# valeoai/rainbow-iqn-apex

Hardware: NVIDIA H100
Metric: learner grad-steps/sec (batch=512, N=N'=64) (higher is better)
Workload: dtype fp16 fwd / bf16 bwd tensor-core products, fp32 accumulate; fp32 elsewhere

## Files before the change

### include/riqn_b200.h

```cpp
#ifndef RIQN_B200_H
#define RIQN_B200_H

#ifdef __cplusplus
extern "C" {
#endif

#define RIQN_B200_ABI_VERSION 1

int riqn_version(void);
long long riqn_launch_count(void);
int riqn_device_ok(void);

typedef struct riqn_dyn_state {
  unsigned long long rng_offset;
  float adam_neg_step_size;
  float adam_sqrt_bc2;
  double is_capacity;
  double is_beta;
} riqn_dyn_state;

typedef struct riqn_conv_geom {
  int B, Cin, H, W;
  int Cout, KH, KW;
  int stride, pad;
  int OH, OW;
  long in_bstride;
} riqn_conv_geom;


int riqn_conv_fwd(const riqn_conv_geom* g, const void* in, int in_is_u8, const float* w, const float* bias,
                  float* col, float* out, void* stream);
int riqn_conv_bwd(const riqn_conv_geom* g, const float* dout, const float* out, const float* col, const float* w,
                  float* dY, float* dcol, float* dw, float* dbias, float* din, void* stream);

int riqn_im2col_f32(const riqn_conv_geom* g, const void* in, int in_is_u8, float* col, void* stream);

int riqn_conv_fwd_tc(const riqn_conv_geom* g, const void* in, int in_is_u8, const void* w_hi, const void* w_lo,
                     const float* bias, void* col_hi, void* col_lo, void* colT_hi, float* out, void* stream);
int riqn_s2d_u8(const riqn_conv_geom* g, const unsigned char* in, void* a_px, void* stream);
int riqn_random_shift(int B, int C, int H, int W, const void* in0, long in0_bstride, const void* in1, long in1_bstride,
                      int is_u8, const int* shifts, void* out, void* stream);
int riqn_conv_fwd_strip(const riqn_conv_geom* g, const void* a_hi, const void* a_lo, const void* w_hi, const void* w_lo,
                        const float* bias, float* out, void* next_hi, void* next_lo, int next_stride, int next_grid,
                        const void* w2_hi, const void* w2_lo, const float* bias2, int share_a, void* stream);
int riqn_conv_bwd_strip(const riqn_conv_geom* g, const float* dout, const float* out, const void* a_hi, const void* w_hi,
                        const int* perm, void* dYg, float* dwp_scratch, float* dw, float* dbias, float* din,
                        float wgrad_scale, void* stream);

int riqn_conv_bwd_tc(const riqn_conv_geom* g, const float* dout, const float* out, const void* colT_hi, const void* wT_hi,
                     void* dY_hi, void* dYT_hi, float* dcol, float* dw, float* dbias, float* din, float wgrad_scale,
                     void* stream);
int riqn_split_bf16_scaled(long rows, int cols, const float* src, float scale, void* hi, void* lo, void* stream);

int riqn_fill_uniform(long n, unsigned long long seed, unsigned long long stream_id, float* out,
                      const riqn_dyn_state* dyn, void* stream);

#define RIQN_RISK_NEUTRAL 0
#define RIQN_RISK_CVAR 1
#define RIQN_RISK_WANG 2
#define RIQN_RISK_CPW 3
#define RIQN_RISK_POW 4
#define RIQN_RISK_NORM 5
int riqn_fill_tau_distorted(long n, unsigned long long seed, unsigned long long stream_id, int measure, float eta,
                            float* out, const riqn_dyn_state* dyn, void* stream);
int riqn_noisy_sample(long n, unsigned long long seed, unsigned long long stream_id, float* out,
                      const riqn_dyn_state* dyn, void* stream);
int riqn_fill_shifts(long n, int pad, unsigned long long seed, unsigned long long stream_id, int* out,
                     const riqn_dyn_state* dyn, void* stream);

int riqn_noisy_compose(int out_features, int in_features, const float* weight_mu, const float* weight_sigma,
                       float* weight_epsilon, const float* eps_in, const float* eps_out, const float* bias_mu,
                       const float* bias_sigma, float* bias_epsilon, float* w_eff, float* b_eff, int training,
                       void* stream);

typedef struct riqn_noisy_layer {
  int out_features, in_features;
  const float* weight_mu;
  const float* weight_sigma;
  float* weight_epsilon;
  const float* bias_mu;
  const float* bias_sigma;
  float* bias_epsilon;
  float* eps_in;
  float* eps_out;
  float* w_eff;
  float* b_eff;
  unsigned long long stream_in, stream_out;
  void* w_hi;
  void* w_lo;
  int w_fp16;
} riqn_noisy_layer;

int riqn_noisy_reset_net(int n_layers, const riqn_noisy_layer* layers, unsigned long long seed, int sample, int training,
                         const riqn_dyn_state* dyn, void* stream);
int riqn_noisy_linear_fwd(long rows, int in_features, int out_features, const float* x, const float* w_eff,
                          const float* b_eff, float* h, void* stream);
int riqn_noisy_linear_dgrad(long rows, int in_features, int out_features, const float* dh, const float* w_eff,
                            float* dx, void* stream);
int riqn_noisy_linear_wgrad(long rows, int in_features, int out_features, const float* dh, const float* x,
                            const float* weight_epsilon, const float* bias_epsilon, float* db_scratch,
                            float* grad_weight_mu, float* grad_weight_sigma, float* grad_bias_mu,
                            float* grad_bias_sigma, void* stream);

int riqn_noisy_bias_grad(long rows, int out_features, const float* dh, const float* bias_epsilon, float* db_scratch,
                         float* grad_bias_mu, float* grad_bias_sigma, void* stream);

int riqn_quantile_embed_fwd(int batch, int num_quantiles, int embed_dim, int feat_dim, const float* tau,
                            const float* feat, const float* iqn_w, const float* iqn_b, float* cosv, float* x,
                            void* stream);
int riqn_quantile_embed_bwd(int batch, int num_quantiles, int embed_dim, int feat_dim, const float* x,
                            const float* feat, const float* cosv, float* dx_inout, float* dfeat, float* grad_iqn_w,
                            float* grad_iqn_b, void* stream);

int riqn_quantile_embed_fwd_tc(int batch, int num_quantiles, int embed_dim, int feat_dim, const float* tau,
                               const float* feat, const void* iqn_w_hi, const void* iqn_w_lo, const float* iqn_b,
                               void* cos_hi, void* cos_lo, void* cos_t_hi, float* x32, void* x_hi, void* x_lo, void* x_hi_t,
                               void* x_lo_t, int x_fp16, void* stream);
int riqn_quantile_embed_bwd_tc(int batch, int num_quantiles, int embed_dim, int feat_dim, const void* x_hi, const void* x_lo,
                               const float* feat, const void* cos_hi, const void* dx, int dx_is_bf16, void* dpre,
                               float* dfeat, float* grad_iqn_w, float* grad_iqn_b, void* stream);

int riqn_dueling_fwd(long rows, int batch, int hidden, int action_space, const float* h, const float* wz,
                     const float* bz, float* q, void* stream);
int riqn_dueling_bwd(long rows, int batch, int hidden, int action_space, const float* h, const float* wz,
                     const float* dtheta, const float* gscale, float gscale_mul, const long long* actions, float* dh,
                     float* dz, void* dz_bf16, void* stream);
int riqn_dueling_bwd_bf16(long rows, int batch, int hidden, int action_space, const float* h, const void* h_bf16,
                          const float* wz,
                          const float* dtheta, const float* gscale, float gscale_mul, const long long* actions, void* dh_hi,
                          void* dh_hi_t,
                          float* dh_colsum, float* dz, void* dz_bf16, void* stream);
int riqn_dueling_bwd_dense(long rows, int batch, int hidden, int action_space, const float* h, const float* wz,
                           const float* grad_q, float* dh, float* dz, void* dz_bf16, void* stream);
int riqn_dueling_bwd_dense_bf16(long rows, int batch, int hidden, int action_space, const float* h, const void* h_bf16,
                                const float* wz, const float* grad_q, void* dh_hi, void* dh_hi_t, float* dh_colsum,
                                float* dz, void* dz_bf16, void* stream);
int riqn_z_wgrad_tc(long rows, int hidden, int action_space, const void* dz_bf16, const void* h_bf16, const float* dz,
                    float* dwz_scratch, float* dbz_scratch, const float* eps_w_zv, const float* eps_b_zv,
                    const float* eps_w_za, const float* eps_b_za, float* g_mu_zv, float* g_sig_zv, float* g_bmu_zv,
                    float* g_bsig_zv, float* g_mu_za, float* g_sig_za, float* g_bmu_za, float* g_bsig_za, void* stream);
int riqn_z_wgrad(long rows, int hidden, int action_space, const float* dz, const float* h, float* dwz_scratch,
                 float* dbz_scratch, const float* eps_w_zv, const float* eps_b_zv, const float* eps_w_za,
                 const float* eps_b_za, float* g_mu_zv, float* g_sig_zv, float* g_bmu_zv, float* g_bsig_zv,
                 float* g_mu_za, float* g_sig_za, float* g_bmu_za, float* g_bsig_za, void* stream);

int riqn_argmax_mean(int batch, int num_quantiles, int action_space, const float* q, long long* a_star, void* stream);
int riqn_iqn_loss_fwd_bwd(int batch, int n_tau, int n_tau_prime, int action_space, const float* q_online,
                          const float* q_target, const float* tau, const long long* actions, const long long* a_star,
                          const float* returns, const float* nonterminals, float gamma_n, float kappa, float* loss,
                          float* dtheta, float* theta_out, float* target_out, void* stream);
int riqn_miqn_loss_fwd_bwd(int batch, int n_tau, int n_tau_prime, int action_space, const float* q_online,
                           const float* q_target, const float* tau, const long long* actions, const float* returns,
                           const float* nonterminals, float gamma_n, float kappa, float alpha, float entropy_tau, float l0,
                           float* loss, float* dtheta, float* theta_out, float* target_out, float* bonus_out, void* stream);

int riqn_value_rescale(long n, const float* x, float eps, int inverse, float* out, void* stream);
int riqn_iqn_loss_fwd_bwd_h(int batch, int n_tau, int n_tau_prime, int action_space, const float* q_online,
                            const float* q_target, const float* tau, const long long* actions, const long long* a_star,
                            const float* returns, const float* nonterminals, float gamma_n, float kappa, float eps,
                            float* loss, float* dtheta, float* theta_out, float* target_out, void* stream);
int riqn_argmax_expected_h(int batch, int n, int action_space, const float* q, const float* w, float eps, float* values,
                           long long* a_star, void* stream);

int riqn_fqf_fractions(int batch, int n, const float* logits, float* tau, float* tau_hat, float* dtau, float* entropy,
                       void* stream);
int riqn_fqf_fraction_bwd(int batch, int n, int action_space, const float* logits, const float* tau, const float* q_hat,
                          const float* q_bnd, const long long* actions, const float* gscale, float gscale_mul,
                          float entropy_coef, float* dlogits, float* loss_out, void* stream);
int riqn_fqf_fraction_wgrad(int batch, int n, int feat_dim, const float* dlogits, const float* feat, float* grad_w,
                            float* grad_b, void* stream);
int riqn_argmax_weighted(int batch, int n, int action_space, const float* q, const float* w, long long* a_star,
                         void* stream);

int riqn_c51_head_fwd(int batch, int action_space, int atoms, const float* zv, const float* za, const float* support,
                      float* p, float* logp, long long* a_star, void* stream);
int riqn_c51_loss_fwd_bwd(int batch, int action_space, int atoms, const float* logp_online, const float* p_target,
                          const long long* actions, const long long* a_star, const float* returns,
                          const float* nonterminals, const float* support, float gamma_n, float v_min, float v_max,
                          float delta_z, float* loss, float* dq, float* m_out, void* stream);
int riqn_c51_loss_fwd_bwd_h(int batch, int action_space, int atoms, const float* logp_online, const float* p_target,
                            const long long* actions, const long long* a_star, const float* returns,
                            const float* nonterminals, const float* support, float gamma_n, float v_min, float v_max,
                            float delta_z, float eps, float* loss, float* dq, float* m_out, void* stream);
int riqn_c51_head_bwd(int batch, int action_space, int atoms, const float* dq, const float* gscale, float gscale_mul,
                      const long long* actions, float* dzv, float* dza, void* stream);
int riqn_c51_head_bwd_dense(int batch, int action_space, int atoms, const float* out, const float* grad_out, int is_log,
                            float* dzv, float* dza, void* stream);

int riqn_qr_head_fwd(int batch, int action_space, int n, const float* zv, const float* za, float* q, void* stream);
int riqn_qr_head_bwd(int batch, int action_space, int n, const float* dtheta, const float* gscale, float gscale_mul,
                     const long long* actions, float* dzv, float* dza, void* stream);
int riqn_qr_head_bwd_dense(int batch, int action_space, int n, const float* grad_q, float* dzv, float* dza, void* stream);
int riqn_zero_f32(float* p, long n, void* stream);
int riqn_relu_mask(long n, const float* act, float* grad, void* stream);
int riqn_linear_fwd_ld(long rows, int in_features, int out_features, const float* x, long ldx, const float* w,
                       const float* bias, float* y, long ldy, int relu, void* stream);
int riqn_linear_dgrad_ld(long rows, int in_features, int out_features, const float* dy, long lddy, const float* w,
                         float* dx, long lddx, void* stream);
int riqn_noisy_wgrad_ld(long rows, int in_features, int out_features, const float* dy, long lddy, const float* x, long ldx,
                        const float* weight_epsilon, float* grad_mu, float* grad_sigma, void* stream);

int riqn_adam_step(long n, float* params, const float* grads, float* exp_avg, float* exp_avg_sq, int step, float lr,
                   float beta1, float beta2, float eps, float grad_scale, const riqn_dyn_state* dyn, void* stream);

int riqn_sumtree_stratified(int n, unsigned long long seed, unsigned long long stream_id, const double* tree,
                            double* values, const riqn_dyn_state* dyn, void* stream);
int riqn_sumtree_sample(int n, long capacity, int actor_capacity, const double* tree, const double* values,
                        const long long* index_actor, int history, int n_step, long long* tree_idx,
                        long long* data_idx, double* priorities, void* stream);
int riqn_sumtree_is_weights(int n, const double* tree, const double* priorities, double current_capacity,
                            double priority_weight, double* w64, float* w32, int* n_nonpositive,
                            const riqn_dyn_state* dyn, void* stream);
int riqn_sumtree_update(int n, long capacity, double* tree, const long long* tree_idx, const float* loss,
                        float priority_exponent, int apply_pow, float* new_priorities, double* diff_scratch,
                        double* max_priority, void* stream);

int riqn_replay_append(int n, int actor_capacity, int id_actor, int start, const unsigned char* frames,
                       const int* timestep, const int* action, const float* reward, const unsigned char* nonterminal,
                       unsigned char* s_frames, int* s_timestep, int* s_action, float* s_reward,
                       unsigned char* s_nonterminal, void* stream);
int riqn_frame_gather(int batch, int actor_capacity, int history, int n_step, const long long* data_idx,
                      const unsigned char* s_frames, const int* s_timestep, const int* s_action, const float* s_reward,
                      const unsigned char* s_nonterminal, const double* gamma_pow, unsigned char* window,
                      long long* actions, float* returns, float* nonterminals, void* stream);

int riqn_split_bf16(long rows, int cols, const float* src, void* hi, void* lo, void* hi_t, void* lo_t, int fp16, void* stream);
typedef struct riqn_split_job {
  const float* src;
  const int* perm;
  int rows, cols;
  float div;
  void* hi;
  void* lo;
  void* hi_t;
} riqn_split_job;
int riqn_split_bf16_multi(int n_jobs, const riqn_split_job* jobs, void* stream);
int riqn_gemm_bf16_tc(int M, int N, int K, const void* a_hi, const void* a_lo, const void* b_hi, const void* b_lo,
                      float* c, long ldc, int epilogue, const float* bias, float* out2, const float* eps, int split_k,
                      void* c_t_bf16, void* c_bf16, int fmt, void* stream);
int riqn_gemm_bf16_tc_mn(int M, int N, int K, const void* a, const void* b_kn, int a_is_km, float* c, long ldc, int epilogue,
                         float* out2, const float* eps, float alpha, int split_k, void* c_bf16, int fmt, void* stream);

int riqn_gemm_f32(int M, int N, int K, const float* A, long sAm, long sAk, const float* B, long sBn, long sBk,
                  float* C, long ldc, void* stream);

#ifdef __cplusplus
}
#endif
#endif
```

### rainbow_iqn_apex_b200/_lib.py

```python
import ctypes as C
import os

import torch

HERE = os.path.dirname(os.path.abspath(__file__))
LIB_PATH = os.path.join(HERE, "libriqn_b200.so")

c_f32p = C.c_void_p
_P = C.c_void_p


class ConvGeom(C.Structure):
    _fields_ = [("B", C.c_int), ("Cin", C.c_int), ("H", C.c_int), ("W", C.c_int), ("Cout", C.c_int),
                ("KH", C.c_int), ("KW", C.c_int), ("stride", C.c_int), ("pad", C.c_int), ("OH", C.c_int),
                ("OW", C.c_int), ("in_bstride", C.c_long)]


class NoisyLayer(C.Structure):
    _fields_ = [("out_features", C.c_int), ("in_features", C.c_int), ("weight_mu", _P), ("weight_sigma", _P),
                ("weight_epsilon", _P), ("bias_mu", _P), ("bias_sigma", _P), ("bias_epsilon", _P), ("eps_in", _P),
                ("eps_out", _P), ("w_eff", _P), ("b_eff", _P), ("stream_in", C.c_ulonglong),
                ("stream_out", C.c_ulonglong), ("w_hi", _P), ("w_lo", _P), ("w_fp16", C.c_int)]


class SplitJob(C.Structure):
    _fields_ = [("src", _P), ("perm", _P), ("rows", C.c_int), ("cols", C.c_int), ("div", C.c_float), ("hi", _P),
                ("lo", _P), ("hi_t", _P)]


SIGNATURES = {
    "riqn_version": [],
    "riqn_device_ok": [],
    "riqn_launch_count": [],
    "riqn_conv_fwd": [C.POINTER(ConvGeom), _P, C.c_int, _P, _P, _P, _P, _P],
    "riqn_conv_bwd": [C.POINTER(ConvGeom), _P, _P, _P, _P, _P, _P, _P, _P, _P, _P],
    "riqn_im2col_f32": [C.POINTER(ConvGeom), _P, C.c_int, _P, _P],
    "riqn_conv_fwd_tc": [C.POINTER(ConvGeom), _P, C.c_int, _P, _P, _P, _P, _P, _P, _P, _P],
    "riqn_conv_bwd_tc": [C.POINTER(ConvGeom), _P, _P, _P, _P, _P, _P, _P, _P, _P, _P, C.c_float, _P],
    "riqn_s2d_u8": [C.POINTER(ConvGeom), _P, _P, _P],
    "riqn_conv_fwd_strip": [C.POINTER(ConvGeom), _P, _P, _P, _P, _P, _P, _P, _P, C.c_int, C.c_int, _P, _P, _P, C.c_int, _P],
    "riqn_conv_bwd_strip": [C.POINTER(ConvGeom), _P, _P, _P, _P, _P, _P, _P, _P, _P, _P, C.c_float, _P],
    "riqn_split_bf16_scaled": [C.c_long, C.c_int, _P, C.c_float, _P, _P, _P],
    "riqn_fill_uniform": [C.c_long, C.c_ulonglong, C.c_ulonglong, _P, _P, _P],
    "riqn_fill_tau_distorted": [C.c_long, C.c_ulonglong, C.c_ulonglong, C.c_int, C.c_float, _P, _P, _P],
    "riqn_noisy_sample": [C.c_long, C.c_ulonglong, C.c_ulonglong, _P, _P, _P],
    "riqn_fill_shifts": [C.c_long, C.c_int, C.c_ulonglong, C.c_ulonglong, _P, _P, _P],
    "riqn_random_shift": [C.c_int] * 4 + [_P, C.c_long, _P, C.c_long, C.c_int, _P, _P, _P],
    "riqn_noisy_compose": [C.c_int, C.c_int, _P, _P, _P, _P, _P, _P, _P, _P, _P, _P, C.c_int, _P],
    "riqn_noisy_reset_net": [C.c_int, C.POINTER(NoisyLayer), C.c_ulonglong, C.c_int, C.c_int, _P, _P],
    "riqn_noisy_linear_fwd": [C.c_long, C.c_int, C.c_int, _P, _P, _P, _P, _P],
    "riqn_noisy_linear_dgrad": [C.c_long, C.c_int, C.c_int, _P, _P, _P, _P],
    "riqn_noisy_linear_wgrad": [C.c_long, C.c_int, C.c_int, _P, _P, _P, _P, _P, _P, _P, _P, _P, _P],
    "riqn_noisy_bias_grad": [C.c_long, C.c_int, _P, _P, _P, _P, _P, _P],
    "riqn_quantile_embed_fwd": [C.c_int, C.c_int, C.c_int, C.c_int, _P, _P, _P, _P, _P, _P, _P],
    "riqn_quantile_embed_fwd_tc": [C.c_int, C.c_int, C.c_int, C.c_int] + [_P] * 13 + [C.c_int, _P],
    "riqn_quantile_embed_bwd_tc": [C.c_int, C.c_int, C.c_int, C.c_int, _P, _P, _P, _P, _P, C.c_int, _P, _P, _P, _P, _P],
    "riqn_quantile_embed_bwd": [C.c_int, C.c_int, C.c_int, C.c_int, _P, _P, _P, _P, _P, _P, _P, _P],
    "riqn_dueling_fwd": [C.c_long, C.c_int, C.c_int, C.c_int, _P, _P, _P, _P, _P],
    "riqn_dueling_bwd": [C.c_long, C.c_int, C.c_int, C.c_int, _P, _P, _P, _P, C.c_float, _P, _P, _P, _P, _P],
    "riqn_dueling_bwd_bf16": [C.c_long, C.c_int, C.c_int, C.c_int] + [_P] * 5 + [C.c_float] + [_P] * 7,
    "riqn_dueling_bwd_dense": [C.c_long, C.c_int, C.c_int, C.c_int, _P, _P, _P, _P, _P, _P, _P],
    "riqn_dueling_bwd_dense_bf16": [C.c_long, C.c_int, C.c_int, C.c_int] + [_P] * 10,
    "riqn_z_wgrad": [C.c_long, C.c_int, C.c_int] + [_P] * 17,
    "riqn_z_wgrad_tc": [C.c_long, C.c_int, C.c_int] + [_P] * 18,
    "riqn_argmax_mean": [C.c_int, C.c_int, C.c_int, _P, _P, _P],
    "riqn_iqn_loss_fwd_bwd": [C.c_int, C.c_int, C.c_int, C.c_int, _P, _P, _P, _P, _P, _P, _P, C.c_float, C.c_float,
                              _P, _P, _P, _P, _P],
    "riqn_miqn_loss_fwd_bwd": [C.c_int] * 4 + [_P] * 6 + [C.c_float] * 5 + [_P] * 6,
    "riqn_fqf_fractions": [C.c_int, C.c_int] + [_P] * 6,
    "riqn_fqf_fraction_bwd": [C.c_int] * 3 + [_P] * 6 + [C.c_float] * 2 + [_P] * 3,
    "riqn_fqf_fraction_wgrad": [C.c_int] * 3 + [_P] * 5,
    "riqn_argmax_weighted": [C.c_int] * 3 + [_P] * 4,
    "riqn_c51_head_fwd":[C.c_int, C.c_int, C.c_int, _P, _P, _P, _P, _P, _P, _P],
    "riqn_c51_loss_fwd_bwd": [C.c_int, C.c_int, C.c_int, _P, _P, _P, _P, _P, _P, _P, C.c_float, C.c_float, C.c_float,
                              C.c_float, _P, _P, _P, _P],
    "riqn_value_rescale": [C.c_long, _P, C.c_float, C.c_int, _P, _P],
    "riqn_iqn_loss_fwd_bwd_h": [C.c_int] * 4 + [_P] * 7 + [C.c_float] * 3 + [_P] * 5,
    "riqn_argmax_expected_h": [C.c_int] * 3 + [_P, _P, C.c_float, _P, _P, _P],
    "riqn_c51_loss_fwd_bwd_h": [C.c_int] * 3 + [_P] * 7 + [C.c_float] * 5 + [_P] * 4,
    "riqn_c51_head_bwd": [C.c_int, C.c_int, C.c_int, _P, _P, C.c_float, _P, _P, _P, _P],
    "riqn_c51_head_bwd_dense": [C.c_int, C.c_int, C.c_int, _P, _P, C.c_int, _P, _P, _P],
    "riqn_qr_head_fwd": [C.c_int] * 3 + [_P] * 4,
    "riqn_qr_head_bwd": [C.c_int] * 3 + [_P, _P, C.c_float, _P, _P, _P, _P],
    "riqn_qr_head_bwd_dense": [C.c_int] * 3 + [_P] * 4,
    "riqn_zero_f32": [_P, C.c_long, _P],
    "riqn_relu_mask": [C.c_long, _P, _P, _P],
    "riqn_linear_fwd_ld": [C.c_long, C.c_int, C.c_int, _P, C.c_long, _P, _P, _P, C.c_long, C.c_int, _P],
    "riqn_linear_dgrad_ld": [C.c_long, C.c_int, C.c_int, _P, C.c_long, _P, _P, C.c_long, _P],
    "riqn_noisy_wgrad_ld": [C.c_long, C.c_int, C.c_int, _P, C.c_long, _P, C.c_long, _P, _P, _P, _P],
    "riqn_adam_step": [C.c_long, _P, _P, _P, _P, C.c_int, C.c_float, C.c_float, C.c_float, C.c_float, C.c_float, _P, _P],
    "riqn_sumtree_stratified": [C.c_int, C.c_ulonglong, C.c_ulonglong, _P, _P, _P, _P],
    "riqn_sumtree_sample": [C.c_int, C.c_long, C.c_int, _P, _P, _P, C.c_int, C.c_int, _P, _P, _P, _P],
    "riqn_sumtree_is_weights": [C.c_int, _P, _P, C.c_double, C.c_double, _P, _P, _P, _P, _P],
    "riqn_sumtree_update": [C.c_int, C.c_long, _P, _P, _P, C.c_float, C.c_int, _P, _P, _P, _P],
    "riqn_replay_append": [C.c_int, C.c_int, C.c_int, C.c_int] + [_P] * 11,
    "riqn_frame_gather": [C.c_int, C.c_int, C.c_int, C.c_int] + [_P] * 12,
    "riqn_split_bf16_multi": [C.c_int, C.POINTER(SplitJob), _P],
    "riqn_split_bf16": [C.c_long, C.c_int, _P, _P, _P, _P, _P, C.c_int, _P],
    "riqn_gemm_bf16_tc": [C.c_int, C.c_int, C.c_int, _P, _P, _P, _P, _P, C.c_long, C.c_int, _P, _P, _P, C.c_int, _P, _P, C.c_int, _P],
    "riqn_gemm_bf16_tc_mn": [C.c_int, C.c_int, C.c_int, _P, _P, C.c_int, _P, C.c_long, C.c_int, _P, _P, C.c_float, C.c_int, _P, C.c_int, _P],
    "riqn_gemm_f32": [C.c_int, C.c_int, C.c_int, _P, C.c_long, C.c_long, _P, C.c_long, C.c_long, _P, C.c_long, _P],
}

_lib = None


class RiqnError(RuntimeError):
    pass


def load():
    global _lib
    if _lib is not None:
        return _lib
    if not os.path.exists(LIB_PATH):
        raise RiqnError(f"{LIB_PATH} is missing: build it with `python -c 'import __graft_entry__ as g; g.build()'` "
                        "(the product has no CPU or PyTorch fallback)")
    lib = C.CDLL(LIB_PATH)
    for name, argtypes in SIGNATURES.items():
        fn = getattr(lib, name)
        fn.argtypes = argtypes
        fn.restype = C.c_longlong if name == "riqn_launch_count" else C.c_int
    if lib.riqn_version() != 1:
        raise RiqnError("ABI version mismatch between _lib.py and libriqn_b200.so")
    _lib = lib
    return lib


def stream():
    return torch.cuda.current_stream().cuda_stream


def ptr(t):
    if t is None:
        return None
    return t.data_ptr()


_timers = None


def time_entry_points(names):
    global _timers
    _timers = {n: [] for n in names} if names else None
    return _timers


def call(name, *args):
    lib = load()
    if _timers is not None and name in _timers:
        e0, e1 = torch.cuda.Event(enable_timing=True), torch.cuda.Event(enable_timing=True)
        e0.record()
        rc = getattr(lib, name)(*args, stream())
        e1.record()
        _timers[name].append((e0, e1, args))
    else:
        rc = getattr(lib, name)(*args, stream())
    if rc != 0:
        raise RiqnError(f"{name} failed with cudaError {rc}")


def launch_count():
    return int(load().riqn_launch_count())


def require_device():
    if not torch.cuda.is_available():
        raise RiqnError("rainbow_iqn_apex_b200 needs a CUDA device (H100, sm_90a); there is no CPU path")
    lib = load()
    ok = lib.riqn_device_ok()
    if ok != 1:
        raise RiqnError(f"libriqn_b200.so holds sm_90a code only; riqn_device_ok() returned {ok}")
```

### rainbow_iqn_apex_b200/c51.py

```python
import torch

from ._lib import call, ptr
from .model import FEAT


def _tc_mode(B):
    from .model import PRECISION
    return PRECISION["fwd"] != "fp32" and PRECISION["bwd"] == "bf16" and B % 8 == 0


def forward(net, x, log=False, keep=None, fresh_weights=False, want_argmax=None, support=None):
    if not fresh_weights:
        net._compose_weights()
    zv, za = hidden_z(net, x, keep=keep)
    B, A, atoms = zv.shape[0], net.action_space, net.atoms
    out = torch.empty(B, A, atoms, device=zv.device)
    if support is None:
        support = net._support(zv.device)
    call("riqn_c51_head_fwd", B, A, atoms, ptr(zv), ptr(za), ptr(support), None if log else ptr(out),
         ptr(out) if log else None, ptr(want_argmax))
    return out


def hidden_z(net, x, keep=None, col_cache=None, feat=None):
    from .model import PRECISION
    if feat is None:
        feat = net.trunk(x, keep, col_cache)
    B = feat.shape[0]
    dev = feat.device
    hid = net.hidden
    nzv, nza = net.fcnoisy_z_v.out_features, net.fcnoisy_z_a.out_features
    h = torch.empty(B, 2 * hid, device=dev)
    x_bf = None
    if _tc_mode(B):
        fwd = PRECISION["fwd"]
        f16, x3 = fwd == "fp16", fwd == "bf16x3"
        x_hi = torch.empty(B, FEAT, dtype=torch.float16 if f16 else torch.bfloat16, device=dev)
        x_lo = torch.empty(B, FEAT, dtype=torch.bfloat16, device=dev) if (x3 or (f16 and keep is not None)) else None
        call("riqn_split_bf16", B, FEAT, ptr(feat), ptr(x_hi), ptr(x_lo), None, None, 1 if f16 else 0)
        call("riqn_gemm_bf16_tc", B, 2 * hid, FEAT, ptr(x_hi), ptr(x_lo) if x3 else None, ptr(net._w_hi),
             ptr(net._w_lo) if x3 else None, ptr(h), 2 * hid, 1, ptr(net._b_eff_h), None, None, 1, None, None, 3 if f16 else 0)
        x_bf = x_lo if f16 else x_hi
    else:
        call("riqn_noisy_linear_fwd", B, FEAT, 2 * hid, ptr(feat), ptr(net._w_eff_h), ptr(net._b_eff_h), ptr(h))
    zv = torch.empty(B, nzv, device=dev)
    za = torch.empty(B, nza, device=dev)
    wz, bz = net._w_eff_z, net._b_eff_z
    hv, ha = h[:, :hid], h[:, hid:]
    call("riqn_linear_fwd_ld", B, hid, nzv, ptr(hv), 2 * hid, ptr(wz), ptr(bz), ptr(zv), nzv, 0)
    wza, bza = wz[nzv:], bz[nzv:]
    call("riqn_linear_fwd_ld", B, hid, nza, ptr(ha), 2 * hid, ptr(wza), ptr(bza), ptr(za), nza, 0)
    if keep is not None:
        keep.update(feat=feat, h=h, B=B, x_bf=x_bf)
    return zv, za


def loss_core(agent, states, actions, returns, next_states, nonterminals, debug=None):
    from .compute_loss_iqn import _as_device_inputs
    states, actions, returns, next_states, nonterminals = _as_device_inputs(
        agent, states, actions, returns, next_states, nonterminals)
    on, tg = agent.online_net, agent.target_net
    B, A, atoms = states.shape[0], agent.action_space, agent.atoms
    dev = states.device
    inj = getattr(agent, "_inject", None)
    if isinstance(inj, list):
        inj = inj.pop(0) if inj else None
    noises = inj.get("noises", (None, None, None)) if inj else (None, None, None)
    on.reset_noise(noises[1])
    a_star = torch.empty(B, dtype=torch.int64, device=dev)
    forward(on, next_states, fresh_weights=True, want_argmax=a_star, support=agent.acting_support)
    tg.reset_noise(noises[2])
    pns = forward(tg, next_states, fresh_weights=True, support=agent.support)
    on.reset_noise(noises[0])
    keep = {}
    log_ps = forward(on, states, log=True, keep=keep, fresh_weights=True, support=agent.support)
    loss = torch.empty(B, device=dev)
    dq = torch.empty(B, atoms, device=dev)
    m_out = torch.empty(B, atoms, device=dev) if debug is not None else None
    args = (ptr(log_ps), ptr(pns), ptr(actions), ptr(a_star), ptr(returns), ptr(nonterminals), ptr(agent.support),
            float(agent.discount ** agent.n), float(agent.Vmin), float(agent.Vmax), float(agent.delta_z))
    eps = getattr(agent, "value_rescaling", None)
    if eps is None:
        call("riqn_c51_loss_fwd_bwd", B, A, atoms, *args, ptr(loss), ptr(dq), ptr(m_out))
    else:
        call("riqn_c51_loss_fwd_bwd_h", B, A, atoms, *args, eps, ptr(loss), ptr(dq), ptr(m_out))
    if debug is not None:
        debug.update(a_star=a_star, m=m_out, log_ps=log_ps)
    version = getattr(on, "_noise_version", 0)

    def backward(gscale, gscale_mul=1.0):
        if getattr(on, "_noise_version", 0) != version:
            raise RuntimeError("the online network's noise was resampled between the C51 loss and its backward")
        gscale = gscale.contiguous().float()
        dzv = torch.empty(B, atoms, device=dev)
        dza = torch.empty(B, A * atoms, device=dev)
        call("riqn_c51_head_bwd", B, A, atoms, ptr(dq), ptr(gscale), float(gscale_mul), ptr(actions), ptr(dzv), ptr(dza))
        _backward_below_head(on, keep, dzv, dza, on.grad_view)

    return loss, backward


def backward_dense(on, keep, out, grad_out, log, gv):
    B, A, atoms = out.shape
    dzv = torch.empty(B, atoms, device=out.device)
    dza = torch.empty(B, A * atoms, device=out.device)
    call("riqn_c51_head_bwd_dense", B, A, atoms, ptr(out), ptr(grad_out), 1 if log else 0, ptr(dzv), ptr(dza))
    _backward_below_head(on, keep, dzv, dza, gv)


def _backward_below_head(on, keep, dzv, dza, gv):
    B, dev = keep["B"], dzv.device
    hid = on.hidden
    hvL, haL, zvL, zaL = on.fcnoisy_h_v, on.fcnoisy_h_a, on.fcnoisy_z_v, on.fcnoisy_z_a
    h = keep["h"]
    dh = torch.empty(B, 2 * hid, device=dev)
    dhv, dha = dh[:, :hid], dh[:, hid:]
    hv, ha = h[:, :hid], h[:, hid:]
    nzv, nza = zvL.out_features, zaL.out_features
    w_z = on._w_eff_z
    wzv, wza = w_z[:nzv], w_z[nzv:]
    call("riqn_linear_dgrad_ld", B, hid, nzv, ptr(dzv), nzv, ptr(wzv), ptr(dhv), 2 * hid)
    call("riqn_linear_dgrad_ld", B, hid, nza, ptr(dza), nza, ptr(wza), ptr(dha), 2 * hid)
    call("riqn_relu_mask", dh.numel(), ptr(h), ptr(dh))
    scratch = torch.empty(max(nza, 2 * hid), device=dev)
    for layer, d, xin in ((zvL, dzv, hv), (zaL, dza, ha)):
        call("riqn_noisy_wgrad_ld", B, hid, layer.out_features, ptr(d), layer.out_features, ptr(xin), 2 * hid,
             ptr(layer.weight_epsilon), ptr(gv(layer.weight_mu)), ptr(gv(layer.weight_sigma)))
        call("riqn_noisy_bias_grad", B, layer.out_features, ptr(d), ptr(layer.bias_epsilon), ptr(scratch),
             ptr(gv(layer.bias_mu)), ptr(gv(layer.bias_sigma)))
    dfeat = torch.empty(B, FEAT, device=dev)
    if keep.get("x_bf") is not None:
        from .model import PRECISION
        dh_bf = torch.empty(B, 2 * hid, dtype=torch.bfloat16, device=dev)
        call("riqn_split_bf16", B, 2 * hid, ptr(dh), ptr(dh_bf), None, None, None, 0)
        w_bf = on._w_lo if PRECISION["fwd"] == "fp16" else on._w_hi
        call("riqn_gemm_bf16_tc_mn", 2 * hid, FEAT, B, ptr(dh_bf), ptr(keep["x_bf"]), 1, ptr(gv(hvL.weight_mu)), FEAT, 3,
             ptr(gv(hvL.weight_sigma)), ptr(hvL.weight_epsilon), 1.0, 1, None, 0)
        call("riqn_noisy_bias_grad", B, 2 * hid, ptr(dh), ptr(hvL.bias_epsilon), ptr(scratch), ptr(gv(hvL.bias_mu)),
             ptr(gv(hvL.bias_sigma)))
        call("riqn_gemm_bf16_tc_mn", B, FEAT, 2 * hid, ptr(dh_bf), ptr(w_bf), 0, ptr(dfeat), FEAT, 0, None, None, 1.0, 1,
             None, 0)
    else:
        call("riqn_noisy_linear_wgrad", B, FEAT, 2 * hid, ptr(dh), ptr(keep["feat"]), ptr(hvL.weight_epsilon),
             ptr(hvL.bias_epsilon), ptr(scratch), ptr(gv(hvL.weight_mu)), ptr(gv(hvL.weight_sigma)), ptr(gv(hvL.bias_mu)),
             ptr(gv(hvL.bias_sigma)))
        call("riqn_noisy_linear_dgrad", B, FEAT, 2 * hid, ptr(dh), ptr(on._w_eff_h), ptr(dfeat))
    on.backward_trunk(keep, dfeat)


class _HeadLoss(torch.autograd.Function):

    @staticmethod
    def forward(ctx, core, agent, states, actions, returns, next_states, nonterminals, debug, *params):
        loss, bw = core(agent, states, actions, returns, next_states, nonterminals, debug=debug)
        ctx.bw, ctx.n_params = bw, len(params)
        return loss

    @staticmethod
    def backward(ctx, grad_loss):
        ctx.bw(grad_loss)
        ctx.bw = None
        return (None,) * (8 + ctx.n_params)


def compute_loss_c51(agent, states, actions, returns, next_states, nonterminals, debug=None):
    if torch.is_grad_enabled():
        params = [p for p in agent.online_net.parameters() if p.requires_grad]
        return _HeadLoss.apply(loss_core, agent, states, actions, returns, next_states, nonterminals, debug, *params)
    loss, _ = loss_core(agent, states, actions, returns, next_states, nonterminals, debug=debug)
    return loss
```

### rainbow_iqn_apex_b200/compute_loss_iqn.py

```python
import ctypes
import math
import numbers

import torch

from ._lib import call, ptr

MUNCHAUSEN_DEFAULTS = {"munchausen_alpha": 0.9, "munchausen_tau": 0.03, "munchausen_l0": -1.0}


def check_munchausen(munchausen, alpha=0.9, entropy_tau=0.03, l0=-1.0, rainbow_only=False, risk=None):
    if isinstance(munchausen, bool) or (isinstance(munchausen, numbers.Integral) and munchausen in (0, 1)):
        if not munchausen:
            return None
    else:
        raise ValueError(f"munchausen must be 0 or 1, got {munchausen!r}")
    vals = []
    for name, v, ok, need in (("munchausen_alpha", alpha, lambda x: x >= 0.0, ">= 0"),
                              ("munchausen_tau", entropy_tau, lambda x: x > 0.0, "> 0"),
                              ("munchausen_l0", l0, lambda x: x <= 0.0, "<= 0")):
        if isinstance(v, bool) or not isinstance(v, numbers.Real):
            raise ValueError(f"{name} must be a real number, got {v!r}")
        f = ctypes.c_float(v).value
        if not (math.isfinite(f) and ok(f)):
            raise ValueError(f"{name} must be finite and {need} (as a float32), got {v!r}")
        vals.append(float(v))
    if rainbow_only:
        raise ValueError("Munchausen targets are implemented for the IQN loss; rainbow_only (C51) does not take them")
    if risk is not None:
        raise ValueError("Munchausen targets have no target action a* to act risk-sensitively on: use the neutral measure")
    return tuple(vals)


VALUE_RESCALING_DEFAULTS = {"value_rescaling_eps": 1e-3}


def check_value_rescaling(value_rescaling, eps=1e-3, munchausen=None):
    if isinstance(value_rescaling, bool) or (isinstance(value_rescaling, numbers.Integral) and value_rescaling in (0, 1)):
        if not value_rescaling:
            return None
    else:
        raise ValueError(f"value_rescaling must be 0 or 1, got {value_rescaling!r}")
    if isinstance(eps, bool) or not isinstance(eps, numbers.Real):
        raise ValueError(f"value_rescaling_eps must be a real number, got {eps!r}")
    f = ctypes.c_float(eps).value
    if not (math.isfinite(f) and f >= 0.0):
        raise ValueError(f"value_rescaling_eps must be finite and >= 0 (as a float32), got {eps!r}")
    if munchausen is not None:
        raise ValueError("value rescaling and Munchausen targets do not combine: set value_rescaling = 0 or munchausen = 0")
    return float(eps)


def greedy_actions(agent, batch, n, q, w=None):
    A = agent.action_space
    a_star = torch.empty(batch, dtype=torch.int64, device=q.device)
    eps = getattr(agent, "value_rescaling", None)
    if eps is not None:
        call("riqn_argmax_expected_h", batch, n, A, ptr(q), ptr(w), eps, None, ptr(a_star))
    elif w is None:
        call("riqn_argmax_mean", batch, n, A, ptr(q), ptr(a_star))
    else:
        call("riqn_argmax_weighted", batch, n, A, ptr(q), ptr(w), ptr(a_star))
    return a_star


def _quantile_loss(agent, B, N, Np, q_on, q_tgt, tau, actions, a_star, returns, nonterminals, loss, dtheta, theta_out,
                   target_out):
    args = (ptr(q_on), ptr(q_tgt), ptr(tau), ptr(actions), ptr(a_star), ptr(returns), ptr(nonterminals),
            float(agent.discount ** agent.n), float(agent.kappa))
    outs = (ptr(loss), ptr(dtheta), ptr(theta_out), ptr(target_out))
    eps = getattr(agent, "value_rescaling", None)
    if eps is None:
        call("riqn_iqn_loss_fwd_bwd", B, N, Np, agent.action_space, *args, *outs)
    else:
        call("riqn_iqn_loss_fwd_bwd_h", B, N, Np, agent.action_space, *args, eps, *outs)


def _as_device_inputs(agent, states, actions, returns, next_states, nonterminals):
    dev = agent.online_net._flat.device

    def frames(x):
        x = x.to(dev)
        return x if x.dtype == torch.uint8 else x.float()

    return (frames(states), actions.to(dev, torch.int64).contiguous(), returns.to(dev, torch.float32).contiguous(),
            frames(next_states), nonterminals.to(dev, torch.float32).contiguous())


def loss_core(agent, states, actions, returns, next_states, nonterminals, keep_graph=True, debug=None):
    states, actions, returns, next_states, nonterminals = _as_device_inputs(
        agent, states, actions, returns, next_states, nonterminals)
    on, tg = agent.online_net, agent.target_net
    B = states.shape[0]
    K, Np, N = agent.num_quantile_samples, agent.num_tau_prime_samples, agent.num_tau_samples
    inj = getattr(agent, "_inject", None)
    if isinstance(inj, list):
        inj = inj.pop(0) if inj else None
    noises = inj.get("noises", (None, None, None)) if inj else (None, None, None)
    taus = inj.get("taus", (None, None, None)) if inj else (None, None, None)
    dev = states.device
    if getattr(agent, "munchausen", None) is not None:
        return _munchausen_core(agent, states, actions, returns, next_states, nonterminals, noises, taus, keep_graph, debug)
    if getattr(agent, "fqf", None) is not None:
        return _fqf_core(agent, states, actions, returns, next_states, nonterminals, noises, keep_graph, debug)

    on.reset_noise(noises[0])
    cache = {}
    pair = on.trunk_pair(tg, next_states) if not on.rainbow_only else None
    f_on, f_tg = pair if pair is not None else (None, None)
    q_sel, tau_sel = on.forward(next_states, K, tau=taus[0], fresh_weights=True, col_cache=cache, feat=f_on,
                                risk=getattr(agent, "risk", None))
    a_star = greedy_actions(agent, B, K, q_sel)
    tg.reset_noise(noises[1])
    q_tgt, _ = tg.forward(next_states, Np, tau=taus[1], fresh_weights=True, col_cache=cache, feat=f_tg)
    on.reset_noise(noises[2])
    keep = {} if keep_graph else None
    q_on, tau = on.forward(states, N, tau=taus[2], keep=keep, fresh_weights=True)

    loss = torch.empty(B, device=dev)
    dtheta = torch.empty(N * B, device=dev)
    theta_out = target_out = None
    if debug is not None:
        theta_out = torch.empty(B, N, device=dev)
        target_out = torch.empty(B, Np, device=dev)
    _quantile_loss(agent, B, N, Np, q_on, q_tgt, tau, actions, a_star, returns, nonterminals, loss, dtheta, theta_out,
                   target_out)
    if debug is not None:
        debug.update(a_star=a_star, theta=theta_out, target=target_out, q_sel=q_sel, q_tgt=q_tgt, q_on=q_on, tau=tau,
                     keep=keep, tau_sel=tau_sel)
    return loss, dtheta, keep, actions


def _munchausen_core(agent, states, actions, returns, next_states, nonterminals, noises, taus, keep_graph, debug):
    on, tg = agent.online_net, agent.target_net
    B, A = states.shape[0], agent.action_space
    Np, N = agent.num_tau_prime_samples, agent.num_tau_samples
    alpha, entropy_tau, l0 = agent.munchausen
    dev = states.device
    tg.reset_noise(noises[0])
    q_tgt, _ = tg.forward(torch.cat((next_states, states)), Np, tau=taus[0], fresh_weights=True)
    on.reset_noise(noises[1])
    keep = {} if keep_graph else None
    q_on, tau = on.forward(states, N, tau=taus[1], keep=keep, fresh_weights=True)

    loss = torch.empty(B, device=dev)
    dtheta = torch.empty(N * B, device=dev)
    theta_out = target_out = bonus_out = None
    if debug is not None:
        theta_out = torch.empty(B, N, device=dev)
        target_out = torch.empty(B, Np, device=dev)
        bonus_out = torch.empty(B, device=dev)
    call("riqn_miqn_loss_fwd_bwd", B, N, Np, A, ptr(q_on), ptr(q_tgt), ptr(tau), ptr(actions), ptr(returns),
         ptr(nonterminals), float(agent.discount ** agent.n), float(agent.kappa), alpha, entropy_tau, l0, ptr(loss),
         ptr(dtheta), ptr(theta_out), ptr(target_out), ptr(bonus_out))
    if debug is not None:
        debug.update(bonus=bonus_out, theta=theta_out, target=target_out, q_tgt=q_tgt, q_on=q_on, tau=tau, keep=keep)
    return loss, dtheta, keep, actions


def _fqf_core(agent, states, actions, returns, next_states, nonterminals, noises, keep_graph, debug):
    on, tg, fnet = agent.online_net, agent.target_net, agent.fraction_net
    B, N = states.shape[0], agent.num_tau_samples
    dev = states.device
    on.reset_noise(noises[0])
    cache = {}
    pair = on.trunk_pair(tg, next_states)
    f_on, f_tg = pair if pair is not None else (on.trunk(next_states, col_cache=cache), None)
    fr_n = fnet.propose(f_on)
    q_sel, _ = on.forward(next_states, N, tau=fr_n["tau_hat"], fresh_weights=True, col_cache=cache, feat=f_on)
    a_star = greedy_actions(agent, B, N, q_sel, fr_n["dtau"])
    keep = {} if keep_graph else None
    feat = on.trunk(states, keep)
    fr = fnet.propose(feat)
    tg.reset_noise(noises[1])
    q_tgt, _ = tg.forward(next_states, N, tau=fr["tau_hat"], fresh_weights=True, col_cache=cache, feat=f_tg)
    on.reset_noise(noises[2])
    q_on, tau_hat = on.forward(states, N, tau=fr["tau_hat"], keep=keep, fresh_weights=True, feat=feat)
    nb = N - 1 if (N - 1) * B % 2 == 0 else N
    q_bnd, _ = on.forward(states, nb, tau=fr["tau"][:, 1:nb + 1].t().contiguous(), fresh_weights=True, feat=feat)

    loss = torch.empty(B, device=dev)
    dtheta = torch.empty(N * B, device=dev)
    theta_out = target_out = None
    if debug is not None:
        theta_out = torch.empty(B, N, device=dev)
        target_out = torch.empty(B, N, device=dev)
    _quantile_loss(agent, B, N, N, q_on, q_tgt, tau_hat, actions, a_star, returns, nonterminals, loss, dtheta, theta_out,
                   target_out)
    if keep is not None:
        keep["fqf"] = dict(fr=fr, q_hat=q_on, q_bnd=q_bnd, actions=actions, debug=debug)
    if debug is not None:
        debug.update(a_star=a_star, theta=theta_out, target=target_out, q_sel=q_sel, q_tgt=q_tgt, q_on=q_on, q_bnd=q_bnd,
                     tau=fr["tau"], tau_hat=fr["tau_hat"], dtau=fr["dtau"], logits=fr["logits"], entropy=fr["entropy"],
                     tau_next=fr_n["tau"], dtau_next=fr_n["dtau"], keep=keep)
    return loss, dtheta, keep, actions


def fraction_backward(agent, keep, gscale, gscale_mul=1.0):
    fk = keep.get("fqf") if keep is not None else None
    if fk is None:
        return
    dlogits, floss = agent.fraction_net.backward(fk["fr"], fk["q_hat"], fk["q_bnd"], fk["actions"], gscale, gscale_mul,
                                                 agent.fqf[1])
    if fk["debug"] is not None:
        fk["debug"].update(dlogits=dlogits, fraction_loss=floss)


class _IQNLoss(torch.autograd.Function):
    @staticmethod
    def forward(ctx, agent, states, actions, returns, next_states, nonterminals, debug, *params):
        loss, dtheta, keep, actions = loss_core(agent, states, actions, returns, next_states, nonterminals,
                                                keep_graph=True, debug=debug)
        ctx.agent, ctx.keep, ctx.dtheta, ctx.actions = agent, keep, dtheta, actions
        ctx.n_params = len(params)
        return loss

    @staticmethod
    def backward(ctx, grad_loss):
        g = grad_loss.contiguous().float()
        ctx.agent.online_net.backward_iqn(ctx.keep, ctx.dtheta, g, ctx.actions)
        fraction_backward(ctx.agent, ctx.keep, g)
        ctx.keep = None
        return (None,) * (7 + ctx.n_params)


def compute_loss_actor_or_learner_iqn(agent, states, actions, returns, next_states, nonterminals, debug=None):
    if torch.is_grad_enabled():
        params = [p for p in agent.online_net.parameters() if p.requires_grad]
        return _IQNLoss.apply(agent, states, actions, returns, next_states, nonterminals, debug, *params)
    loss, _, _, _ = loss_core(agent, states, actions, returns, next_states, nonterminals, keep_graph=False, debug=debug)
    return loss
```

### rainbow_iqn_apex_b200/csrc/conv.cu

```cuda
#include "common.cuh"
#include "gemm.h"
#include "../../include/riqn_b200.h"

namespace riqn {

template <typename T>
__device__ __forceinline__ float load_px(const T* p);
template <>
__device__ __forceinline__ float load_px<uint8_t>(const uint8_t* p) { return (float)(*p) / 255.0f; }
template <>
__device__ __forceinline__ float load_px<float>(const float* p) { return *p; }

template <typename T>
__global__ void im2col_kernel(riqn_conv_geom g, const T* __restrict__ in, float* __restrict__ col) {
  const int K = g.Cin * g.KH * g.KW;
  const long total = (long)g.B * g.OH * g.OW * K;
  for (long idx = (long)blockIdx.x * blockDim.x + threadIdx.x; idx < total; idx += (long)gridDim.x * blockDim.x) {
    const int k = (int)(idx % K);
    const long m = idx / K;
    const int kw = k % g.KW, kh = (k / g.KW) % g.KH, c = k / (g.KW * g.KH);
    const int ow = (int)(m % g.OW), oh = (int)((m / g.OW) % g.OH), b = (int)(m / ((long)g.OW * g.OH));
    const int ih = oh * g.stride + kh - g.pad, iw = ow * g.stride + kw - g.pad;
    float v = 0.f;
    if (ih >= 0 && ih < g.H && iw >= 0 && iw < g.W) v = load_px<T>(&in[(long)b * g.in_bstride + ((long)c * g.H + ih) * g.W + iw]);
    col[idx] = v;
  }
}

__global__ void conv_dy_kernel(int B, int Cout, int ohw, const float* __restrict__ dout,
                               const float* __restrict__ out, float* __restrict__ dY) {
  const long total = (long)B * Cout * ohw;
  for (long idx = (long)blockIdx.x * blockDim.x + threadIdx.x; idx < total; idx += (long)gridDim.x * blockDim.x) {
    const int p = (int)(idx % ohw);
    const int c = (int)((idx / ohw) % Cout);
    const long b = idx / ((long)ohw * Cout);
    const float v = out[idx] > 0.f ? dout[idx] : 0.f;
    dY[(b * ohw + p) * Cout + c] = v;
  }
}

__global__ void col2im_kernel(riqn_conv_geom g, const float* __restrict__ dcol, float* __restrict__ din) {
  const int K = g.Cin * g.KH * g.KW;
  const long total = (long)g.B * g.Cin * g.H * g.W;
  for (long idx = (long)blockIdx.x * blockDim.x + threadIdx.x; idx < total; idx += (long)gridDim.x * blockDim.x) {
    const int iw = (int)(idx % g.W), ih = (int)((idx / g.W) % g.H);
    const int c = (int)((idx / ((long)g.W * g.H)) % g.Cin);
    const long b = idx / ((long)g.W * g.H * g.Cin);
    float acc = 0.f;
    for (int kh = 0; kh < g.KH; ++kh) {
      const int t = ih + g.pad - kh;
      if (t < 0 || t % g.stride) continue;
      const int oh = t / g.stride;
      if (oh >= g.OH) continue;
      for (int kw = 0; kw < g.KW; ++kw) {
        const int u = iw + g.pad - kw;
        if (u < 0 || u % g.stride) continue;
        const int ow = u / g.stride;
        if (ow >= g.OW) continue;
        acc += dcol[((b * g.OH + oh) * g.OW + ow) * K + (c * g.KH + kh) * g.KW + kw];
      }
    }
    din[idx] = acc;
  }
}

__global__ void col2im_tile_kernel(riqn_conv_geom g, int CC, const float* __restrict__ dcol, float* __restrict__ din) {
  extern __shared__ float acc[];
  const int K = g.Cin * g.KH * g.KW, khw = g.KH * g.KW, ohw = g.OH * g.OW, hw = g.H * g.W;
  const int chunks = g.Cin / CC;
  const long b = blockIdx.x / chunks;
  const int c0 = (blockIdx.x % chunks) * CC;
  for (int i = threadIdx.x; i < CC * hw; i += blockDim.x) acc[i] = 0.f;
  __syncthreads();
  const int per_row = CC * khw;
  const float* base = dcol + b * ohw * (long)K + (long)c0 * khw;
  for (int e = threadIdx.x; e < ohw * per_row; e += blockDim.x) {
    const int m = e / per_row, j = e - m * per_row;
    const int c = j / khw, r = j - c * khw;
    const int kh = r / g.KW, kw = r - kh * g.KW;
    const int oh = m / g.OW, ow = m - oh * g.OW;
    const int ih = oh * g.stride + kh - g.pad, iw = ow * g.stride + kw - g.pad;
    if (ih >= 0 && ih < g.H && iw >= 0 && iw < g.W) atomicAdd(&acc[c * hw + ih * g.W + iw], base[(long)m * K + j]);
  }
  __syncthreads();
  float* out = din + (b * g.Cin + c0) * hw;
  for (int i = threadIdx.x; i < CC * hw; i += blockDim.x) out[i] = acc[i];
}

static int col2im(const riqn_conv_geom* g, const float* dcol, float* din, cudaStream_t s) {
  const int hw = g->H * g->W;
  int CC = g->Cin;
  while (CC > 1 && ((long)CC * hw * 4 > 16 * 1024 || g->Cin % CC)) --CC;
  if ((long)CC * hw * 4 <= 48 * 1024) {
    col2im_tile_kernel<<<g->B * (g->Cin / CC), 256, (size_t)CC * hw * 4, s>>>(*g, CC, dcol, din);
  } else {
    long total = (long)g->B * g->Cin * hw;
    long blocks = (total + 255) / 256;
    col2im_kernel<<<(int)(blocks > 32L * riqn_sms() ? 32L * riqn_sms() : blocks), 256, 0, s>>>(*g, dcol, din);
  }
  return (int)cudaGetLastError();
}

__global__ void colsum_part_kernel(long M, int N, const float* __restrict__ X, float* __restrict__ part, int rows_per_block) {
  __shared__ float upper[128];
  const int n = blockIdx.x * 128 + (threadIdx.x & 127);
  const int half = threadIdx.x >> 7;
  const long r0 = (long)blockIdx.y * rows_per_block;
  const long r1 = min(M, r0 + rows_per_block);
  float acc = 0.f;
  if (n < N)
    for (long r = r0 + half; r < r1; r += 2) acc += X[r * N + n];
  if (half) upper[threadIdx.x & 127] = acc;
  __syncthreads();
  if (!half && n < N) part[(long)blockIdx.y * N + n] = acc + upper[threadIdx.x];
}

int colsum_add(long M, int N, const float* X, float* out, cudaStream_t s) {
  int rows_per_block = 256;
  dim3 grid((N + 127) / 128, (unsigned)((M + rows_per_block - 1) / rows_per_block));
  StreamScratch part;
  RIQN_CUDA(part.alloc((size_t)grid.y * N, s));
  colsum_part_kernel<<<grid, 256, 0, s>>>(M, N, X, part.p, rows_per_block);
  RIQN_LAUNCH_CHECK();
  return sum_slots_add((int)grid.y, N, part.p, out, s);
}

using bf16 = __nv_bfloat16;

template <typename T>
__device__ __forceinline__ float im2col_at(const riqn_conv_geom& g, const T* __restrict__ in, long m, int k) {
  const int kw = k % g.KW, kh = (k / g.KW) % g.KH, c = k / (g.KW * g.KH);
  const int ow = (int)(m % g.OW), oh = (int)((m / g.OW) % g.OH);
  const long b = m / ((long)g.OW * g.OH);
  const int ih = oh * g.stride + kh - g.pad, iw = ow * g.stride + kw - g.pad;
  if (ih < 0 || ih >= g.H || iw < 0 || iw >= g.W) return 0.f;
  return load_px<T>(&in[b * g.in_bstride + ((long)c * g.H + ih) * g.W + iw]);
}

__device__ __forceinline__ void pack8(const float (&x)[8], uint4& hi, uint4& lo) {
  uint32_t h[4], l[4];
#pragma unroll
  for (int t = 0; t < 8; t += 2) {
    const bf16 h0 = __float2bfloat16_rn(x[t]), h1 = __float2bfloat16_rn(x[t + 1]);
    const bf16 l0 = __float2bfloat16_rn(x[t] - __bfloat162float(h0)), l1 = __float2bfloat16_rn(x[t + 1] - __bfloat162float(h1));
    h[t / 2] = (uint32_t)__bfloat16_as_ushort(h0) | ((uint32_t)__bfloat16_as_ushort(h1) << 16);
    l[t / 2] = (uint32_t)__bfloat16_as_ushort(l0) | ((uint32_t)__bfloat16_as_ushort(l1) << 16);
  }
  hi = make_uint4(h[0], h[1], h[2], h[3]);
  lo = make_uint4(l[0], l[1], l[2], l[3]);
}

template <typename T>
__global__ void im2col_bf16_kernel(riqn_conv_geom g, const T* __restrict__ in, bf16* __restrict__ hi, bf16* __restrict__ lo) {
  const int K = g.Cin * g.KH * g.KW, K8 = K / 8;
  const long total = (long)g.B * g.OH * g.OW * K8;
  for (long idx = (long)blockIdx.x * blockDim.x + threadIdx.x; idx < total; idx += (long)gridDim.x * blockDim.x) {
    const int k0 = (int)(idx % K8) * 8;
    const long m = idx / K8;
    const int ow = (int)(m % g.OW), oh = (int)((m / g.OW) % g.OH);
    const long b = m / ((long)g.OW * g.OH);
    int kw = k0 % g.KW, kh = (k0 / g.KW) % g.KH, c = k0 / (g.KW * g.KH);
    const T* base = in + b * g.in_bstride;
    const int ih0 = oh * g.stride - g.pad, iw0 = ow * g.stride - g.pad;
    float x[8];
#pragma unroll
    for (int t = 0; t < 8; ++t) {
      const int ih = ih0 + kh, iw = iw0 + kw;
      x[t] = (ih >= 0 && ih < g.H && iw >= 0 && iw < g.W) ? load_px<T>(&base[((long)c * g.H + ih) * g.W + iw]) : 0.f;
      if (++kw == g.KW) { kw = 0; if (++kh == g.KH) { kh = 0; ++c; } }
    }
    uint4 h, l;
    pack8(x, h, l);
    *reinterpret_cast<uint4*>(hi + m * K + k0) = h;
    if (lo) *reinterpret_cast<uint4*>(lo + m * K + k0) = l;
  }
}

__global__ void im2col_bf16_u8_kernel(riqn_conv_geom g, const uint8_t* __restrict__ in, bf16* __restrict__ hi, bf16* __restrict__ lo) {
  __shared__ uint32_t lut[256];
  {
    const float x = (float)threadIdx.x / 255.0f;
    const bf16 h = __float2bfloat16_rn(x);
    const bf16 l = __float2bfloat16_rn(x - __bfloat162float(h));
    if (threadIdx.x < 256) lut[threadIdx.x] = (uint32_t)__bfloat16_as_ushort(h) | ((uint32_t)__bfloat16_as_ushort(l) << 16);
  }
  __syncthreads();
  const int K = g.Cin * g.KH * g.KW, K8 = K / 8;
  const long total = (long)g.B * g.OH * g.OW * K8;
  for (long idx = (long)blockIdx.x * blockDim.x + threadIdx.x; idx < total; idx += (long)gridDim.x * blockDim.x) {
    const int k0 = (int)(idx % K8) * 8;
    const long m = idx / K8;
    const int ow = (int)(m % g.OW), oh = (int)((m / g.OW) % g.OH);
    const long b = m / ((long)g.OW * g.OH);
    int kw = k0 % g.KW, kh = (k0 / g.KW) % g.KH, c = k0 / (g.KW * g.KH);
    const uint8_t* base = in + b * g.in_bstride;
    const int ih0 = oh * g.stride - g.pad, iw0 = ow * g.stride - g.pad;
    uint32_t e[8];
#pragma unroll
    for (int t = 0; t < 8; ++t) {
      const int ih = ih0 + kh, iw = iw0 + kw;
      e[t] = (ih >= 0 && ih < g.H && iw >= 0 && iw < g.W) ? lut[base[((long)c * g.H + ih) * g.W + iw]] : 0u;
      if (++kw == g.KW) { kw = 0; if (++kh == g.KH) { kh = 0; ++c; } }
    }
    uint4 h, l;
    h.x = (e[0] & 0xffffu) | (e[1] << 16); h.y = (e[2] & 0xffffu) | (e[3] << 16);
    h.z = (e[4] & 0xffffu) | (e[5] << 16); h.w = (e[6] & 0xffffu) | (e[7] << 16);
    l.x = (e[0] >> 16) | (e[1] & 0xffff0000u); l.y = (e[2] >> 16) | (e[3] & 0xffff0000u);
    l.z = (e[4] >> 16) | (e[5] & 0xffff0000u); l.w = (e[6] >> 16) | (e[7] & 0xffff0000u);
    *reinterpret_cast<uint4*>(hi + m * K + k0) = h;
    if (lo) *reinterpret_cast<uint4*>(lo + m * K + k0) = l;
  }
}

__global__ void __launch_bounds__(256) im2col_f32_staged_kernel(riqn_conv_geom g, const float* __restrict__ in,
                                                                bf16* __restrict__ hi, bf16* __restrict__ lo) {
  extern __shared__ __align__(16) uint32_t simg[];
  const int chw = g.Cin * g.H * g.W, K = g.Cin * g.KH * g.KW, K8 = K / 8, ohw = g.OH * g.OW;
  const long b = blockIdx.x;
  const float4* src = reinterpret_cast<const float4*>(in + b * g.in_bstride);
  for (int i = threadIdx.x; i < chw / 4; i += blockDim.x) {
    const float4 v = __ldg(src + i);
    const float x[4] = {v.x, v.y, v.z, v.w};
    uint32_t w[4];
#pragma unroll
    for (int t = 0; t < 4; ++t) {
      const bf16 h = __float2bfloat16_rn(x[t]);
      const bf16 l = __float2bfloat16_rn(x[t] - __bfloat162float(h));
      w[t] = (uint32_t)__bfloat16_as_ushort(h) | ((uint32_t)__bfloat16_as_ushort(l) << 16);
    }
    reinterpret_cast<uint4*>(simg)[i] = make_uint4(w[0], w[1], w[2], w[3]);
  }
  __syncthreads();
  const int hw = g.H * g.W;
  for (int item = threadIdx.x; item < ohw * K8; item += blockDim.x) {
    const int m = item / K8, k0 = (item - m * K8) * 8;
    const int oh = m / g.OW, ow = m - oh * g.OW;
    int kw = k0 % g.KW, kh = (k0 / g.KW) % g.KH, c = k0 / (g.KW * g.KH);
    const int ih0 = oh * g.stride - g.pad, iw0 = ow * g.stride - g.pad;
    uint32_t e[8];
#pragma unroll
    for (int t = 0; t < 8; ++t) {
      const int ih = ih0 + kh, iw = iw0 + kw;
      e[t] = ((unsigned)ih < (unsigned)g.H && (unsigned)iw < (unsigned)g.W) ? simg[c * hw + ih * g.W + iw] : 0u;
      if (++kw == g.KW) { kw = 0; if (++kh == g.KH) { kh = 0; ++c; } }
    }
    const long o = (b * ohw + m) * K + k0;
    *reinterpret_cast<uint4*>(hi + o) = make_uint4(__byte_perm(e[0], e[1], 0x5410), __byte_perm(e[2], e[3], 0x5410),
                                                   __byte_perm(e[4], e[5], 0x5410), __byte_perm(e[6], e[7], 0x5410));
    if (lo)
      *reinterpret_cast<uint4*>(lo + o) = make_uint4(__byte_perm(e[0], e[1], 0x7632), __byte_perm(e[2], e[3], 0x7632),
                                                     __byte_perm(e[4], e[5], 0x7632), __byte_perm(e[6], e[7], 0x7632));
  }
}

template <typename T>
__global__ void im2col_bf16_t_kernel(riqn_conv_geom g, const T* __restrict__ in, bf16* __restrict__ hiT) {
  const int K = g.Cin * g.KH * g.KW;
  const long M = (long)g.B * g.OH * g.OW, M8 = M / 8;
  const long total = M8 * K;
  for (long idx = (long)blockIdx.x * blockDim.x + threadIdx.x; idx < total; idx += (long)gridDim.x * blockDim.x) {
    const long m0 = (idx % M8) * 8;
    const int k = (int)(idx / M8);
    const int kw = k % g.KW, kh = (k / g.KW) % g.KH, c = k / (g.KW * g.KH);
    int ow = (int)(m0 % g.OW), oh = (int)((m0 / g.OW) % g.OH);
    long b = m0 / ((long)g.OW * g.OH);
    float x[8];
#pragma unroll
    for (int t = 0; t < 8; ++t) {
      const int ih = oh * g.stride + kh - g.pad, iw = ow * g.stride + kw - g.pad;
      x[t] = (ih >= 0 && ih < g.H && iw >= 0 && iw < g.W)
                 ? load_px<T>(&in[b * g.in_bstride + ((long)c * g.H + ih) * g.W + iw]) : 0.f;
      if (++ow == g.OW) { ow = 0; if (++oh == g.OH) { oh = 0; ++b; } }
    }
    uint4 h, l;
    pack8(x, h, l);
    *reinterpret_cast<uint4*>(hiT + (long)k * M + m0) = h;
  }
}

__global__ void conv_dy_bf16_kernel(int B, int Cout, int ohw, const float* __restrict__ dout, const float* __restrict__ out,
                                    bf16* __restrict__ dY, bf16* __restrict__ dYT, float* __restrict__ dbias_part) {
  const int c = blockIdx.y;
  const long M = (long)B * ohw;
  float acc = 0.f;
  for (long i = (long)blockIdx.x * blockDim.x + threadIdx.x; i < M; i += (long)gridDim.x * blockDim.x) {
    const long b = i / ohw;
    const int p = (int)(i - b * ohw);
    const long src = (b * Cout + c) * ohw + p;
    const float v = out[src] > 0.f ? dout[src] : 0.f;
    acc += v;
    const bf16 h = __float2bfloat16_rn(v);
    if (dY) dY[i * Cout + c] = h;
    dYT[(long)c * M + i] = h;
  }
  acc = warp_sum(acc);
  __shared__ float red[32];
  if ((threadIdx.x & 31) == 0) red[threadIdx.x >> 5] = acc;
  __syncthreads();
  if (threadIdx.x < 32) {
    float v = threadIdx.x < (blockDim.x >> 5) ? red[threadIdx.x] : 0.f;
    v = warp_sum(v);
    if (threadIdx.x == 0) dbias_part[(long)blockIdx.x * Cout + c] = v;
  }
}

__global__ void __launch_bounds__(256) conv_dy_tile_kernel(int B, int Cout, int ohw, const float* __restrict__ dout,
                                                           const float* __restrict__ out, bf16* __restrict__ dY,
                                                           bf16* __restrict__ dYT, float* __restrict__ dbias_part) {
  __shared__ __align__(16) unsigned short tile[64][66];
  __shared__ float bsum[64];
  const long M = (long)B * ohw;
  const int lane = threadIdx.x & 31, warp = threadIdx.x >> 5;
  if (threadIdx.x < 64) bsum[threadIdx.x] = 0.f;
  __syncthreads();
  const long n_tiles = (M + 63) / 64;
  for (long tix = blockIdx.x; tix < n_tiles; tix += gridDim.x) {
    const long m0 = tix * 64;
    long src0[2];
    bool ok[2];
#pragma unroll
    for (int h = 0; h < 2; ++h) {
      const long m = m0 + lane + 32 * h;
      ok[h] = m < M;
      const long b = ok[h] ? m / ohw : 0;
      src0[h] = b * Cout * ohw + (ok[h] ? m - b * ohw : 0);
    }
    for (int c = warp; c < Cout; c += 8) {
      float acc = 0.f;
#pragma unroll
      for (int h = 0; h < 2; ++h) {
        float v = 0.f;
        if (ok[h]) {
          const long src = src0[h] + (long)c * ohw;
          v = out[src] > 0.f ? dout[src] : 0.f;
        }
        const bf16 hb = __float2bfloat16_rn(v);
        if (ok[h]) dYT[(long)c * M + m0 + lane + 32 * h] = hb;
        tile[lane + 32 * h][c] = __bfloat16_as_ushort(hb);
        acc += v;
      }
      acc = warp_sum(acc);
      if (lane == 0) bsum[c] += acc;
    }
    __syncthreads();
    if (dY) {
      const int ppr = Cout >> 3;
      for (int idx = threadIdx.x; idx < 64 * ppr; idx += blockDim.x) {
        const int r = idx / ppr, pc = idx - r * ppr;
        if (m0 + r < M) {
          const uint32_t* w = reinterpret_cast<const uint32_t*>(&tile[r][pc * 8]);
          *reinterpret_cast<uint4*>(dY + (m0 + r) * Cout + pc * 8) = make_uint4(w[0], w[1], w[2], w[3]);
        }
      }
    }
    __syncthreads();
  }
  if (threadIdx.x < Cout) dbias_part[(long)blockIdx.x * Cout + threadIdx.x] = bsum[threadIdx.x];
}

__global__ void __launch_bounds__(256) s2d_u8_kernel(riqn_conv_geom g, int G, const uint8_t* __restrict__ in,
                                                     bf16* __restrict__ a_px) {
  extern __shared__ __align__(16) uint8_t img[];
  const int chw = g.Cin * g.H * g.W, s = g.stride, ss = s * s, Kc = ss * g.Cin, K8 = Kc / 8;
  const long b = blockIdx.x;
  const uint4* src = reinterpret_cast<const uint4*>(in + b * g.in_bstride);
  for (int i = threadIdx.x; i < chw / 16; i += blockDim.x) reinterpret_cast<uint4*>(img)[i] = src[i];
  __syncthreads();
  const bool fast = s == 4 && g.pad == 1 && (g.W & 3) == 0 && (G - 1) * 4 + 2 < g.W && (G - 1) * 4 + 2 < g.H;
  if (fast) {
    const uint32_t* img32 = reinterpret_cast<const uint32_t*>(img);
    const int wpr = g.W >> 2;
    auto cvt2 = [](uint32_t w, uint32_t sa, uint32_t sb) -> uint32_t {
      const float fa = __uint_as_float(__byte_perm(w, 0x4B000000u, sa)) - 8388608.0f;
      const float fb = __uint_as_float(__byte_perm(w, 0x4B000000u, sb)) - 8388608.0f;
      return __byte_perm(__float_as_uint(fa), __float_as_uint(fb), 0x7632);
    };
    for (int item = threadIdx.x; item < G * G * K8; item += blockDim.x) {
      const int r = item / K8, q = item - r * K8;
      const int gy = r / G, gx = r - gy * G, c = q >> 1, iy0 = (q & 1) * 2;
      uint32_t o[4];
#pragma unroll
      for (int h = 0; h < 2; ++h) {
        const int y = gy * 4 + iy0 + h - 1;
        uint32_t w0 = 0u, w1 = 0u;
        if (y >= 0) {
          const uint32_t* rowp = img32 + (c * g.H + y) * wpr + gx;
          w0 = gx > 0 ? rowp[-1] : 0u;
          w1 = rowp[0];
        }
        const uint32_t a = __byte_perm(w0, w1, 0x0043);
        o[2 * h] = cvt2(a, 0x7650, 0x7651);
        o[2 * h + 1] = cvt2(w1, 0x7651, 0x7652);
      }
      *reinterpret_cast<uint4*>(a_px + (b * G * G + r) * Kc + q * 8) = make_uint4(o[0], o[1], o[2], o[3]);
    }
    return;
  }
  for (int item = threadIdx.x; item < G * G * K8; item += blockDim.x) {
    const int r = item / K8, k0 = (item - r * K8) * 8;
    const int gy = r / G, gx = r - gy * G;
    uint32_t e[8];
#pragma unroll
    for (int t = 0; t < 8; ++t) {
      const int k = k0 + t, c = k / ss, rem = k - c * ss, iy = rem / s, ix = rem - iy * s;
      const int y = gy * s + iy - g.pad, x = gx * s + ix - g.pad;
      e[t] = ((unsigned)y < (unsigned)g.H && (unsigned)x < (unsigned)g.W)
                 ? __float_as_uint((float)img[(c * g.H + y) * g.W + x]) >> 16 : 0u;
    }
    *reinterpret_cast<uint4*>(a_px + (b * G * G + r) * Kc + k0) =
        make_uint4(e[0] | (e[1] << 16), e[2] | (e[3] << 16), e[4] | (e[5] << 16), e[6] | (e[7] << 16));
  }
}

static inline int grid_for(long total) {
  long b = (total + 255) / 256;
  return (int)(b > 32L * riqn_sms() ? 32L * riqn_sms() : (b < 1 ? 1 : b));
}

}

using namespace riqn;

RIQN_API int riqn_conv_fwd(const riqn_conv_geom* g, const void* in, int in_is_u8, const float* w, const float* bias,
                           float* col, float* out, void* stream) {
  riqn::note_launches(2);
  cudaStream_t s = (cudaStream_t)stream;
  const long M = (long)g->B * g->OH * g->OW;
  const int K = g->Cin * g->KH * g->KW;
  if (in_is_u8) im2col_kernel<uint8_t><<<grid_for(M * K), 256, 0, s>>>(*g, (const uint8_t*)in, col);
  else im2col_kernel<float><<<grid_for(M * K), 256, 0, s>>>(*g, (const float*)in, col);
  RIQN_LAUNCH_CHECK();
  EpiArgs e;
  e.bias = bias;
  e.ohw = g->OH * g->OW;
  return gemm_f32((int)M, g->Cout, K, col, K, 1, w, K, 1, out, g->Cout, EPI_BIAS_RELU_NCHW, e, 1, s);
}

RIQN_API int riqn_im2col_f32(const riqn_conv_geom* g, const void* in, int in_is_u8, float* col, void* stream) {
  riqn::note_launches(1);
  cudaStream_t s = (cudaStream_t)stream;
  const long M = (long)g->B * g->OH * g->OW;
  const int K = g->Cin * g->KH * g->KW;
  if (in_is_u8) im2col_kernel<uint8_t><<<grid_for(M * K), 256, 0, s>>>(*g, (const uint8_t*)in, col);
  else im2col_kernel<float><<<grid_for(M * K), 256, 0, s>>>(*g, (const float*)in, col);
  return (int)cudaGetLastError();
}

RIQN_API int riqn_conv_bwd(const riqn_conv_geom* g, const float* dout, const float* out, const float* col,
                           const float* w, float* dY, float* dcol, float* dw, float* dbias, float* din, void* stream) {
  riqn::note_launches(din ? 5 : 3);
  cudaStream_t s = (cudaStream_t)stream;
  const long M = (long)g->B * g->OH * g->OW;
  const int K = g->Cin * g->KH * g->KW;
  const int ohw = g->OH * g->OW;
  conv_dy_kernel<<<grid_for(M * g->Cout), 256, 0, s>>>(g->B, g->Cout, ohw, dout, out, dY);
  RIQN_LAUNCH_CHECK();
  int rc = colsum_add(M, g->Cout, dY, dbias, s);
  if (rc) return rc;
  EpiArgs e;
  const int tiles = ((g->Cout + 127) / 128) * ((K + 127) / 128);
  int split = (2 * riqn_sms() + tiles - 1) / tiles;
  if ((long)split * 64 > M) split = (int)((M + 63) / 64);
  rc = gemm_f32(g->Cout, K, (int)M, dY, 1, g->Cout, col, 1, K, dw, K, EPI_ATOMIC, e, split, s);
  if (rc) return rc;
  if (din) {
    rc = gemm_f32((int)M, K, g->Cout, dY, g->Cout, 1, w, 1, K, dcol, K, EPI_STORE, e, 1, s);
    if (rc) return rc;
    rc = col2im(g, dcol, din, s);
    if (rc) return rc;
  }
  return 0;
}


RIQN_API int riqn_conv_fwd_tc(const riqn_conv_geom* g, const void* in, int in_is_u8, const void* w_hi, const void* w_lo,
                              const float* bias, void* col_hi, void* col_lo, void* colT_hi, float* out, void* stream) {
  riqn::note_launches(colT_hi ? 3 : 2);
  cudaStream_t s = (cudaStream_t)stream;
  const long M = (long)g->B * g->OH * g->OW;
  const int K = g->Cin * g->KH * g->KW;
  if (K % 8 || (colT_hi && M % 8)) return (int)cudaErrorInvalidValue;
  if (in_is_u8) im2col_bf16_u8_kernel<<<grid_for(M * K / 8), 256, 0, s>>>(*g, (const uint8_t*)in, (bf16*)col_hi, (bf16*)col_lo);
  else {
    const int chw = g->Cin * g->H * g->W;
    if (chw % 4 == 0 && g->in_bstride % 4 == 0 && (reinterpret_cast<uintptr_t>(in) & 15) == 0 && chw * 4 <= 96 * 1024) {
      static PerDeviceOnce attr_once;
      const int attr_dev = PerDeviceOnce::device();
      if (!attr_once.done[attr_dev]) {
        RIQN_CUDA(cudaFuncSetAttribute(im2col_f32_staged_kernel, cudaFuncAttributeMaxDynamicSharedMemorySize, 96 * 1024));
        attr_once.done[attr_dev] = true;
      }
      im2col_f32_staged_kernel<<<g->B, 256, (size_t)chw * 4, s>>>(*g, (const float*)in, (bf16*)col_hi, (bf16*)col_lo);
    } else {
      im2col_bf16_kernel<float><<<grid_for(M * K / 8), 256, 0, s>>>(*g, (const float*)in, (bf16*)col_hi, (bf16*)col_lo);
    }
  }
  RIQN_LAUNCH_CHECK();
  if (colT_hi) {
    if (in_is_u8) im2col_bf16_t_kernel<uint8_t><<<grid_for(M * K / 8), 256, 0, s>>>(*g, (const uint8_t*)in, (bf16*)colT_hi);
    else im2col_bf16_t_kernel<float><<<grid_for(M * K / 8), 256, 0, s>>>(*g, (const float*)in, (bf16*)colT_hi);
    RIQN_LAUNCH_CHECK();
  }
  TcExtra ex;
  ex.ohw = g->OH * g->OW;
  return gemm_bf16_tc((int)M, g->Cout, K, (const bf16*)col_hi, (const bf16*)col_lo, (const bf16*)w_hi,
                      col_lo ? (const bf16*)w_lo : nullptr, out, g->Cout, TC_BIAS_RELU_NCHW, bias, nullptr, nullptr, 1, s, &ex);
}

__global__ void __launch_bounds__(256) conv_dy_grid_kernel(int B, int Cout, int OH, int OW, int G,
                                                           const float* __restrict__ dout, const float* __restrict__ out,
                                                           bf16* __restrict__ dYg, float* __restrict__ dbias_part) {
  __shared__ __align__(16) unsigned short tile[64][66];
  __shared__ float bsum[64];
  const long Mg = (long)B * G * G;
  const int lane = threadIdx.x & 31, warp = threadIdx.x >> 5, ohw = OH * OW, gg = G * G;
  if (threadIdx.x < 64) bsum[threadIdx.x] = 0.f;
  __syncthreads();
  const long n_tiles = (Mg + 63) / 64;
  for (long tix = blockIdx.x; tix < n_tiles; tix += gridDim.x) {
    const long m0 = tix * 64;
    long src0[2];
    bool ok[2];
#pragma unroll
    for (int h = 0; h < 2; ++h) {
      const long m = m0 + lane + 32 * h;
      const long b = m / gg;
      const int rem = (int)(m - b * gg), gy = rem / G, gx = rem - gy * G;
      ok[h] = m < Mg && gy < OH && gx < OW;
      src0[h] = ok[h] ? b * Cout * ohw + gy * OW + gx : 0;
    }
    for (int c0 = warp; c0 < Cout; c0 += 32) {
      float o_[4][2], d_[4][2];
#pragma unroll
      for (int u = 0; u < 4; ++u)
#pragma unroll
        for (int h = 0; h < 2; ++h) {
          const int c = c0 + 8 * u;
          const bool on = ok[h] && c < Cout;
          const long src = src0[h] + (long)c * ohw;
          o_[u][h] = on ? __ldg(out + src) : 0.f;
          d_[u][h] = on ? __ldg(dout + src) : 0.f;
        }
#pragma unroll
      for (int u = 0; u < 4; ++u) {
        const int c = c0 + 8 * u;
        if (c < Cout) {
          float acc = 0.f;
#pragma unroll
          for (int h = 0; h < 2; ++h) {
            const float v = o_[u][h] > 0.f ? d_[u][h] : 0.f;
            tile[lane + 32 * h][c] = __bfloat16_as_ushort(__float2bfloat16_rn(v));
            acc += v;
          }
          acc = warp_sum(acc);
          if (lane == 0) bsum[c] += acc;
        }
      }
    }
    __syncthreads();
    const int ppr = Cout >> 3;
    for (int idx = threadIdx.x; idx < 64 * ppr; idx += blockDim.x) {
      const int r = idx / ppr, pc = idx - r * ppr;
      if (m0 + r < Mg) {
        const uint32_t* w = reinterpret_cast<const uint32_t*>(&tile[r][pc * 8]);
        *reinterpret_cast<uint4*>(dYg + (m0 + r) * Cout + pc * 8) = make_uint4(w[0], w[1], w[2], w[3]);
      }
    }
    __syncthreads();
  }
  if (threadIdx.x < Cout) dbias_part[(long)blockIdx.x * Cout + threadIdx.x] = bsum[threadIdx.x];
}

__global__ void unpermute_add_kernel(int Cout, int K, const float* __restrict__ dwp, const int* __restrict__ perm,
                                     float* __restrict__ dw, const bf16* __restrict__ w_hi, bf16* __restrict__ w_s) {
  const int idx = blockIdx.x * blockDim.x + threadIdx.x;
  if (idx >= Cout * K) return;
  const int c = idx / K, kp = idx - c * K;
  const long o = (long)c * K + perm[kp];
  dw[o] += dwp[idx];
  if (w_s) w_s[idx] = w_hi[o];
}

static int strip_params(const riqn_conv_geom* g, int* t, int* G, int* kc) {
  if (g->KH != g->KW || g->stride < 1 || g->KH % g->stride) return 1;
  *t = g->KH / g->stride;
  *G = g->OH + *t - 1;
  const int Kc = g->stride * g->stride * g->Cin;
  if (g->OH != g->OW || Kc % 64 || g->OH != (g->H + 2 * g->pad - g->KH) / g->stride + 1) return 1;
  *kc = Kc / 64;
  return 0;
}

RIQN_API int riqn_s2d_u8(const riqn_conv_geom* g, const unsigned char* in, void* a_px, void* stream) {
  riqn::note_launches(1);
  int t, G, kc;
  const int chw = g->Cin * g->H * g->W;
  if (strip_params(g, &t, &G, &kc) || chw % 16 || g->in_bstride % 16 || (reinterpret_cast<uintptr_t>(in) & 15) ||
      chw > 96 * 1024)
    return (int)cudaErrorInvalidValue;
  static PerDeviceOnce attr_once;
  const int attr_dev = PerDeviceOnce::device();
  if (!attr_once.done[attr_dev]) {
    RIQN_CUDA(cudaFuncSetAttribute(s2d_u8_kernel, cudaFuncAttributeMaxDynamicSharedMemorySize, 96 * 1024));
    attr_once.done[attr_dev] = true;
  }
  s2d_u8_kernel<<<g->B, 256, chw, (cudaStream_t)stream>>>(*g, G, in, (bf16*)a_px);
  return (int)cudaGetLastError();
}

RIQN_API int riqn_conv_fwd_strip(const riqn_conv_geom* g, const void* a_hi, const void* a_lo, const void* w_hi,
                                 const void* w_lo, const float* bias, float* out, void* next_hi, void* next_lo,
                                 int next_stride, int next_grid, const void* w2_hi, const void* w2_lo, const float* bias2,
                                 int share_a, void* stream) {
  riqn::note_launches(1);
  int t, G, kc;
  if (strip_params(g, &t, &G, &kc) || g->Cout > 64 || (next_hi && (next_stride < 1 || next_grid < 1)))
    return (int)cudaErrorInvalidValue;
  TcExtra ex;
  if (w2_hi != nullptr) {
    const long rows = (long)g->B * G * G;
    if ((g->B & 1) || (rows / 2) % 128 || bias2 == nullptr || (w_lo != nullptr) != (w2_lo != nullptr)) return (int)cudaErrorInvalidValue;
    ex.grp_mt = (int)(rows / 2 / 128);
    ex.b2_hi = (const bf16*)w2_hi; ex.b2_lo = (const bf16*)w2_lo; ex.bias2 = bias2;
    if (share_a) { ex.a_wrap = 1; ex.a_rows = rows / 2; }
  }
  ex.strip_t = t; ex.strip_G = G; ex.strip_kc = kc;
  ex.cv_oh = g->OH; ex.cv_ow = g->OW;
  ex.nx_hi = (bf16*)next_hi; ex.nx_lo = (bf16*)next_lo; ex.nx_s = next_stride; ex.nx_G = next_grid;
  return gemm_bf16_tc(g->B * G * G, g->Cout, g->Cin * g->KH * g->KW, (const bf16*)a_hi, (const bf16*)a_lo, (const bf16*)w_hi,
                      (const bf16*)w_lo, out, g->Cout, TC_CONV, bias, nullptr, nullptr, 1, (cudaStream_t)stream, &ex);
}

RIQN_API int riqn_conv_bwd_strip(const riqn_conv_geom* g, const float* dout, const float* out, const void* a_hi,
                                 const void* w_hi, const int* perm, void* dYg, float* dwp_scratch, float* dw, float* dbias,
                                 float* din, float wgrad_scale, void* stream) {
  riqn::note_launches(din ? 5 : 4);
  cudaStream_t s = (cudaStream_t)stream;
  int t, G, kc;
  if (strip_params(g, &t, &G, &kc) || g->Cout > 64 || g->Cout % 8 ||
      (din && (g->pad != 0 || g->H != g->W || G * g->stride != g->H)))
    return (int)cudaErrorInvalidValue;
  const long Mg = (long)g->B * G * G;
  const int K = g->Cin * g->KH * g->KW;
  const long tiles = (Mg + 63) / 64;
  const int dy_grid = (int)(tiles < 4L * riqn_sms() ? tiles : 4L * riqn_sms());
  StreamScratch dbias_part;
  RIQN_CUDA(dbias_part.alloc((size_t)dy_grid * g->Cout, s));
  conv_dy_grid_kernel<<<dy_grid, 256, 0, s>>>(g->B, g->Cout, g->OH, g->OW, G, dout, out, (bf16*)dYg, dbias_part.p);
  RIQN_LAUNCH_CHECK();
  if (int rc_ = sum_slots_add(dy_grid, g->Cout, dbias_part.p, dbias, s)) return rc_;
  RIQN_CUDA(cudaMemsetAsync(dwp_scratch, 0, sizeof(float) * g->Cout * K, s));
  TcExtra ex;
  ex.mn_major = 3;
  ex.wg_t = t; ex.wg_G = G; ex.wg_kc = kc;
  ex.alpha = wgrad_scale;
  const int n_tiles = (K + 127) / 128;
  const int split = tc_pick_split(n_tiles, (Mg + 63) / 64);
  int rc = gemm_bf16_tc(g->Cout, K, (int)Mg, (const bf16*)dYg, nullptr, (const bf16*)a_hi, nullptr, dwp_scratch, K, TC_ATOMIC,
                        nullptr, nullptr, nullptr, split, s, &ex);
  if (rc) return rc;
  StreamScratch w_s;
  if (din) RIQN_CUDA(w_s.alloc(((size_t)g->Cout * K + 1) / 2, s));
  unpermute_add_kernel<<<(g->Cout * K + 255) / 256, 256, 0, s>>>(g->Cout, K, dwp_scratch, perm, dw, (const bf16*)w_hi,
                                                                 (bf16*)w_s.p);
  RIQN_LAUNCH_CHECK();
  if (din) {
    TcExtra dg;
    dg.strip_t = t; dg.strip_G = G;
    dg.ci_cin = g->Cin; dg.ci_h = g->H; dg.ci_w = g->W; dg.ci_stride = g->stride;
    rc = gemm_bf16_tc((int)Mg, kc * 64, g->Cout, (const bf16*)dYg, nullptr, (const bf16*)w_s.p, nullptr, din, 0,
                      TC_CONV_DGRAD, nullptr, nullptr, nullptr, 1, s, &dg);
    if (rc) return rc;
  }
  return 0;
}

RIQN_API int riqn_conv_bwd_tc(const riqn_conv_geom* g, const float* dout, const float* out, const void* colT_hi,
                              const void* wT_hi, void* dY_hi, void* dYT_hi, float* dcol, float* dw, float* dbias, float* din,
                              float wgrad_scale, void* stream) {
  riqn::note_launches(din ? 4 : 2);
  cudaStream_t s = (cudaStream_t)stream;
  const long M = (long)g->B * g->OH * g->OW;
  const int K = g->Cin * g->KH * g->KW;
  const int ohw = g->OH * g->OW;
  if (M % 8 || g->Cout % 8) return (int)cudaErrorInvalidValue;
  const long tiles = (M + 63) / 64;
  const int slots = g->Cout <= 64 ? (int)(tiles < 4L * riqn_sms() ? tiles : 4L * riqn_sms()) : (int)((M + 256 * 8 - 1) / (256 * 8));
  StreamScratch dbias_part;
  RIQN_CUDA(dbias_part.alloc((size_t)slots * g->Cout, s));
  if (g->Cout <= 64) {
    conv_dy_tile_kernel<<<slots, 256, 0, s>>>(g->B, g->Cout, ohw, dout, out, din ? (bf16*)dY_hi : nullptr, (bf16*)dYT_hi,
                                              dbias_part.p);
  } else {
    dim3 grid((unsigned)slots, g->Cout);
    conv_dy_bf16_kernel<<<grid, 256, 0, s>>>(g->B, g->Cout, ohw, dout, out, din ? (bf16*)dY_hi : nullptr, (bf16*)dYT_hi,
                                             dbias_part.p);
  }
  RIQN_LAUNCH_CHECK();
  if (int rc_ = sum_slots_add(slots, g->Cout, dbias_part.p, dbias, s)) return rc_;
  const int n_tiles = (K + 127) / 128;
  int split = (riqn_sms() + n_tiles - 1) / n_tiles;
  TcExtra ex;
  ex.alpha = wgrad_scale;
  int rc = gemm_bf16_tc(g->Cout, K, (int)M, (const bf16*)dYT_hi, nullptr, (const bf16*)colT_hi, nullptr, dw, K, TC_ATOMIC,
                        nullptr, nullptr, nullptr, split, s, &ex);
  if (rc) return rc;
  if (din) {
    if (g->pad == 0) {
      RIQN_CUDA(cudaMemsetAsync(din, 0, sizeof(float) * (size_t)g->B * g->Cin * g->H * g->W, s));
      TcExtra ci;
      ci.ohw = ohw;
      ci.ci_h = g->H; ci.ci_w = g->W; ci.ci_cin = g->Cin; ci.ci_kh = g->KH; ci.ci_kw = g->KW;
      ci.ci_stride = g->stride; ci.ci_ow = g->OW;
      rc = gemm_bf16_tc((int)M, K, g->Cout, (const bf16*)dY_hi, nullptr, (const bf16*)wT_hi, nullptr, din, K, TC_COL2IM,
                        nullptr, nullptr, nullptr, 1, s, &ci);
      if (rc) return rc;
    } else {
      rc = gemm_bf16_tc((int)M, K, g->Cout, (const bf16*)dY_hi, nullptr, (const bf16*)wT_hi, nullptr, dcol, K, TC_STORE,
                        nullptr, nullptr, nullptr, 1, s, nullptr);
      if (rc) return rc;
      rc = col2im(g, dcol, din, s);
      if (rc) return rc;
    }
  }
  return 0;
}
```

### rainbow_iqn_apex_b200/model.py

```python
import ctypes
import math
import numbers
import os
import weakref

import torch
from torch import nn

from . import _lib
from ._lib import ConvGeom, NoisyLayer, SplitJob, call, ptr

FEAT = 3136
_EAGER_STREAMS = 1 << 39
_ALIGN = 64

PRECISION = {"fwd": os.environ.get("RIQN_FWD_PRECISION", "fp16"), "bwd": os.environ.get("RIQN_BWD_PRECISION", "bf16")}
WGRAD_SPLIT_K = int(os.environ.get("RIQN_WGRAD_SPLIT_K", "4"))


def set_precision(fwd=None, bwd=None):
    for k, v in (("fwd", fwd), ("bwd", bwd)):
        if v is not None:
            if v not in ("bf16x3", "bf16", "fp32") + (("fp16",) if k == "fwd" else ()):
                raise ValueError(v)
            PRECISION[k] = v
    if PRECISION["fwd"] == "fp16" and PRECISION["bwd"] != "bf16":
        raise ValueError("the fp16 forward pairs with the bf16 backward (it reads the bf16 images written beside the fp16 ones)")


RISK_MEASURES = {"neutral": 0, "cvar": 1, "wang": 2, "cpw": 3, "pow": 4, "norm": 5}


def check_risk(risk):
    if risk is None:
        return None
    try:
        measure, eta = risk
    except (TypeError, ValueError):
        raise ValueError(f"risk must be None or a (measure, eta) pair, got {risk!r}") from None
    name = measure.lower() if isinstance(measure, str) else None
    if name not in RISK_MEASURES:
        raise ValueError(f"unknown risk measure {measure!r} (one of {', '.join(RISK_MEASURES)})")
    if name == "neutral":
        return None
    if isinstance(eta, bool) or not isinstance(eta, numbers.Real):
        raise ValueError(f"the {name} risk measure needs a real eta, got {eta!r}")
    e = ctypes.c_float(eta).value
    ok = {"cvar": 0.0 < e <= 1.0, "wang": math.isfinite(e), "cpw": 0.0 < e < math.inf, "pow": math.isfinite(e),
          "norm": 1.0 <= e <= 32.0 and e == int(e)}[name]
    if not ok:
        need = {"cvar": "0 < eta <= 1", "wang": "a finite eta", "cpw": "eta > 0", "pow": "a finite eta",
                "norm": "an integer eta in [1, 32]"}[name]
        raise ValueError(f"the {name} risk measure needs {need}, got eta={eta!r}")
    return name, float(eta)


def _small_x3():
    return PRECISION["fwd"] in ("bf16x3", "fp16")


class NoisyLinear(nn.Module):

    def __init__(self, in_features, out_features, std_init, disable_cuda=False):
        super().__init__()
        self.disable_cuda = disable_cuda
        self.in_features = in_features
        self.out_features = out_features
        self.std_init = std_init
        self.weight_mu = nn.Parameter(torch.empty(out_features, in_features))
        self.weight_sigma = nn.Parameter(torch.empty(out_features, in_features))
        self.register_buffer("weight_epsilon", torch.zeros(out_features, in_features))
        self.bias_mu = nn.Parameter(torch.empty(out_features))
        self.bias_sigma = nn.Parameter(torch.empty(out_features))
        self.register_buffer("bias_epsilon", torch.zeros(out_features))
        self._eps_in = None
        self._eps_out = None
        self._w_eff = None
        self._b_eff = None
        self._noise_calls = 0
        self._calls_in_step = 0
        self._dyn = None
        self._layer_id = 0
        self.reset_parameters()

    def reset_parameters(self):
        mu_range = 1 / math.sqrt(self.in_features)
        self.weight_mu.data.uniform_(-mu_range, mu_range)
        self.weight_sigma.data.fill_(self.std_init / math.sqrt(self.in_features))
        self.bias_mu.data.uniform_(-mu_range, mu_range)
        self.bias_sigma.data.fill_(self.std_init / math.sqrt(self.out_features))

    def _ensure_scratch(self):
        dev = self.weight_mu.device
        if self._eps_in is None or self._eps_in.device != dev:
            self._eps_in = torch.empty(self.in_features, device=dev)
            self._eps_out = torch.empty(self.out_features, device=dev)
        if self._w_eff is None or self._w_eff.device != dev:
            self._w_eff = torch.empty(self.out_features, self.in_features, device=dev)
            self._b_eff = torch.empty(self.out_features, device=dev)

    def reset_noise(self, eps_in=None, eps_out=None, seed=None):
        self._ensure_scratch()
        if eps_in is None:
            if seed is None:
                seed = int(torch.randint(0, 2 ** 62, (1,)).item())
            dyn = self._dyn
            idx = self._calls_in_step if dyn is not None else self._noise_calls
            base = (self._layer_id << 40) + 2 * idx + (0 if dyn is not None else _EAGER_STREAMS)
            call("riqn_noisy_sample", self.in_features, seed, base, ptr(self._eps_in), dyn.ptr() if dyn else None)
            call("riqn_noisy_sample", self.out_features, seed, base + 1, ptr(self._eps_out), dyn.ptr() if dyn else None)
            self._noise_calls += 1
            self._calls_in_step += 1
        else:
            self._eps_in.copy_(eps_in)
            self._eps_out.copy_(eps_out)
        self._compose(resample=True)

    def _compose(self, resample=False):
        self._ensure_scratch()
        call("riqn_noisy_compose", self.out_features, self.in_features, ptr(self.weight_mu), ptr(self.weight_sigma),
             ptr(self.weight_epsilon), ptr(self._eps_in) if resample else None,
             ptr(self._eps_out) if resample else None, ptr(self.bias_mu), ptr(self.bias_sigma),
             ptr(self.bias_epsilon), ptr(self._w_eff), ptr(self._b_eff), 1 if self.training else 0)

    def forward(self, input):
        if torch.is_grad_enabled() and (input.requires_grad or any(p.requires_grad for p in self.parameters())):
            return _NoisyLinearFn.apply(self, input, self.weight_mu, self.weight_sigma, self.bias_mu, self.bias_sigma)
        return self._forward(input)

    def _forward(self, input):
        self._compose()
        x = input.contiguous().float()
        out = torch.empty(x.shape[0], self.out_features, device=x.device)
        call("riqn_gemm_f32", x.shape[0], self.out_features, self.in_features, ptr(x), self.in_features, 1,
             ptr(self._w_eff), self.in_features, 1, ptr(out), self.out_features)
        return out + self._b_eff


def _strip_perm(cin, k, stride, first):
    t = k // stride
    idx = []
    for dy in range(t):
        for dx in range(t):
            if first:
                order = [(c, iy, ix) for c in range(cin) for iy in range(stride) for ix in range(stride)]
            else:
                order = [(c, iy, ix) for iy in range(stride) for ix in range(stride) for c in range(cin)]
            idx += [c * k * k + (stride * dy + iy) * k + (stride * dx + ix) for c, iy, ix in order]
    return torch.tensor(idx, dtype=torch.long)


def _geom(batch, cin, h, cout, k, stride, pad, in_bstride=None):
    oh = (h + 2 * pad - k) // stride + 1
    return ConvGeom(batch, cin, h, h, cout, k, k, stride, pad, oh, oh, in_bstride if in_bstride else cin * h * h)


def _strip_block(g):
    return g.OH + g.KH // g.stride - 1, g.stride * g.stride * g.Cin


class DQN(nn.Module):

    def __init__(self, args, action_space):
        super().__init__()
        self.rainbow_only = args.rainbow_only
        self.action_space = action_space
        self.device = args.device
        self.disable_cuda = args.disable_cuda
        self.history = args.history_length
        self.hidden = args.hidden_size
        if self.hidden != 512:
            raise ValueError("the sm_90a kernels are specialised for hidden_size == 512")
        self.conv1 = nn.Conv2d(args.history_length, 32, 8, stride=4, padding=1)
        self.conv2 = nn.Conv2d(32, 64, 4, stride=2)
        self.conv3 = nn.Conv2d(64, 64, 3)
        from . import qr
        self.num_quantiles = qr.check_qr(getattr(args, "qr_dqn", 0), getattr(args, "num_tau_samples", None),
                                         action_space, rainbow_only=self.rainbow_only)
        self.qr_dqn = self.num_quantiles is not None
        if self.qr_dqn:
            zv, za = self.num_quantiles, action_space * self.num_quantiles
        elif self.rainbow_only:
            self.atoms = args.atoms
            self._v_min, self._v_max = args.V_min, args.V_max
            zv, za = self.atoms, action_space * self.atoms
        else:
            self.quantile_embedding_dim = args.quantile_embedding_dim
            self.iqn_fc = nn.Linear(self.quantile_embedding_dim, FEAT)
            zv, za = 1, action_space
        kw = dict(std_init=args.noisy_std, disable_cuda=args.disable_cuda)
        self.fcnoisy_h_v = NoisyLinear(FEAT, args.hidden_size, **kw)
        self.fcnoisy_h_a = NoisyLinear(FEAT, args.hidden_size, **kw)
        self.fcnoisy_z_v = NoisyLinear(args.hidden_size, zv, **kw)
        self.fcnoisy_z_a = NoisyLinear(args.hidden_size, za, **kw)
        for i, m in enumerate((self.fcnoisy_h_v, self.fcnoisy_h_a, self.fcnoisy_z_v, self.fcnoisy_z_a)):
            m._layer_id = i + 1
        self._tau_calls = 0
        self._tau_in_step = 0
        self._shift_calls = self._shift_in_step = 0
        self._dyn = None
        self._tau_stream_offset = 0
        self._rng_seed = int(torch.randint(0, 2 ** 62, (1,)).item())
        self._param_version = 0
        self._flatten()
        self.register_load_state_dict_post_hook(lambda module, _incompatible: module._params_changed())
        if self._flat.is_cuda:
            self.reset_noise()

    def _embeds(self):
        return not (self.rainbow_only or self.qr_dqn)

    def _param_groups_in_arena_order(self):
        g = [[self.conv1.weight], [self.conv1.bias], [self.conv2.weight], [self.conv2.bias],
             [self.conv3.weight], [self.conv3.bias]]
        if self._embeds():
            g += [[self.iqn_fc.weight], [self.iqn_fc.bias]]
        hv, ha, zv, za = self.fcnoisy_h_v, self.fcnoisy_h_a, self.fcnoisy_z_v, self.fcnoisy_z_a
        g += [[hv.weight_mu, ha.weight_mu], [hv.weight_sigma, ha.weight_sigma],
              [hv.bias_mu, ha.bias_mu], [hv.bias_sigma, ha.bias_sigma],
              [zv.weight_mu, za.weight_mu], [zv.weight_sigma, za.weight_sigma],
              [zv.bias_mu, za.bias_mu], [zv.bias_sigma, za.bias_sigma]]
        return g

    def _flatten(self):
        groups = self._param_groups_in_arena_order()
        dev = groups[0][0].device
        total = 0
        offsets = []
        for grp in groups:
            total = (total + _ALIGN - 1) // _ALIGN * _ALIGN
            for p in grp:
                offsets.append(total)
                total += p.numel()
        total = (total + _ALIGN - 1) // _ALIGN * _ALIGN
        flat = torch.zeros(total, device=dev, dtype=torch.float32)
        flat_grad = torch.zeros(total, device=dev, dtype=torch.float32)
        i = 0
        self._offsets = {}
        for grp in groups:
            for p in grp:
                off, n = offsets[i], p.numel()
                flat[off:off + n].copy_(p.data.reshape(-1).float())
                p.data = flat[off:off + n].view(p.shape)
                p.grad = flat_grad[off:off + n].view(p.shape)
                self._offsets[id(p)] = off
                p._riqn_owner = weakref.ref(self)
                p._riqn_offset = off
                i += 1
        self._flat, self._flat_grad = flat, flat_grad
        self._params_changed()
        hv, ha, zv, za = self.fcnoisy_h_v, self.fcnoisy_h_a, self.fcnoisy_z_v, self.fcnoisy_z_a
        eg = [[(hv, "weight_epsilon"), (ha, "weight_epsilon")], [(hv, "bias_epsilon"), (ha, "bias_epsilon")],
              [(zv, "weight_epsilon"), (za, "weight_epsilon")], [(zv, "bias_epsilon"), (za, "bias_epsilon")]]
        etotal, eoffs = 0, []
        for grp in eg:
            etotal = (etotal + _ALIGN - 1) // _ALIGN * _ALIGN
            for m, name in grp:
                eoffs.append(etotal)
                etotal += m._buffers[name].numel()
        eflat = torch.zeros(etotal + _ALIGN, device=dev, dtype=torch.float32)
        i = 0
        for grp in eg:
            for m, name in grp:
                old = m._buffers[name]
                n = old.numel()
                eflat[eoffs[i]:eoffs[i] + n].copy_(old.reshape(-1).float())
                m._buffers[name] = eflat[eoffs[i]:eoffs[i] + n].view(old.shape)
                i += 1
        self._eps_flat = eflat
        hid = self.hidden
        nz = zv.out_features + za.out_features
        self._w_eff_h = torch.empty(2 * hid, FEAT, device=dev)
        self._b_eff_h = torch.empty(2 * hid, device=dev)
        self._w_eff_z = torch.empty(nz, hid, device=dev)
        self._b_eff_z = torch.empty(nz, device=dev)
        hv._w_eff, ha._w_eff = self._w_eff_h[:hid], self._w_eff_h[hid:]
        hv._b_eff, ha._b_eff = self._b_eff_h[:hid], self._b_eff_h[hid:]
        zv._w_eff, za._w_eff = self._w_eff_z[:zv.out_features], self._w_eff_z[zv.out_features:]
        zv._b_eff, za._b_eff = self._b_eff_z[:zv.out_features], self._b_eff_z[zv.out_features:]
        for m in (hv, ha, zv, za):
            m._eps_in = torch.empty(m.in_features, device=dev)
            m._eps_out = torch.empty(m.out_features, device=dev)

    def _apply(self, fn, *a, **k):
        out = super()._apply(fn, *a, **k)
        self._flatten()
        if self._flat.is_cuda:
            self.reset_noise()
        return out

    def _params_changed(self):
        self._static_ops_dirty = True
        self._param_version += 1

    def zero_grad(self, set_to_none=False):
        if self._flat_grad.is_cuda:
            call("riqn_zero_f32", ptr(self._flat_grad), self._flat_grad.numel())
        else:
            self._flat_grad.zero_()
        for grp in self._param_groups_in_arena_order():
            for p in grp:
                if p.grad is None or p.grad.data_ptr() != self._flat_grad.data_ptr() + 4 * self._offsets[id(p)]:
                    off = self._offsets[id(p)]
                    p.grad = self._flat_grad[off:off + p.numel()].view(p.shape)

    def grad_view(self, p):
        off = self._offsets[id(p)]
        return self._flat_grad[off:off + p.numel()].view(p.shape)

    def noisy_layers(self):
        return [(n, m) for n, m in self.named_children() if "fcnoisy" in n]

    def reset_noise(self, noise=None):
        self._noise_version = getattr(self, "_noise_version", 0) + 1
        self._composed_training = self.training
        layers = self.noisy_layers()
        if not self._flat.is_cuda or any(m.in_features % 4 for _, m in layers):
            for name, module in layers:
                if noise is not None:
                    e_in, e_out = noise[name]
                    module.reset_noise(e_in.to(self._flat.device), e_out.to(self._flat.device))
                else:
                    module.reset_noise(seed=self._rng_seed)
            self._refresh_tc_operands()
            return
        desc = self._noisy_desc()
        for k, (name, m) in enumerate(layers):
            if noise is not None:
                e_in, e_out = noise[name]
                m._eps_in.copy_(e_in)
                m._eps_out.copy_(e_out)
            else:
                idx = m._calls_in_step if m._dyn is not None else m._noise_calls
                base = (m._layer_id << 40) + 2 * idx + (0 if m._dyn is not None else _EAGER_STREAMS)
                desc[k].stream_in, desc[k].stream_out = base, base + 1
                m._noise_calls += 1
                m._calls_in_step += 1
        dyn = layers[0][1]._dyn
        seed = self._rng_seed
        if seed is None:
            seed = int(torch.randint(0, 2 ** 62, (1,)).item())
        call("riqn_noisy_reset_net", len(layers), desc, seed, 0 if noise is not None else 1, 1 if self.training else 0,
             dyn.ptr() if (dyn is not None and noise is None) else None)
        self._refresh_tc_operands(h_done=self._fuse_h_images())

    def _noisy_desc(self):
        layers = self.noisy_layers()
        fuse = self._fuse_h_images()
        w_hi = getattr(self, "_w_hi", None) if fuse else None
        f16 = PRECISION["fwd"] == "fp16"
        key = tuple(m.weight_mu.data_ptr() for _, m in layers) + (self._flat.data_ptr(), w_hi.data_ptr() if fuse else 0, f16)
        if getattr(self, "_noisy_desc_key", None) != key:
            arr = (NoisyLayer * len(layers))()
            for k, (name, m) in enumerate(layers):
                if fuse and name in ("fcnoisy_h_v", "fcnoisy_h_a"):
                    row0 = 0 if name == "fcnoisy_h_v" else self.hidden
                    arr[k].w_hi = self._w_hi.data_ptr() + row0 * FEAT * 2
                    arr[k].w_lo = self._w_lo.data_ptr() + row0 * FEAT * 2
                    arr[k].w_fp16 = 1 if f16 else 0
                m._ensure_scratch()
                d = arr[k]
                d.out_features, d.in_features = m.out_features, m.in_features
                d.weight_mu, d.weight_sigma, d.weight_epsilon = ptr(m.weight_mu), ptr(m.weight_sigma), ptr(m.weight_epsilon)
                d.bias_mu, d.bias_sigma, d.bias_epsilon = ptr(m.bias_mu), ptr(m.bias_sigma), ptr(m.bias_epsilon)
                d.eps_in, d.eps_out, d.w_eff, d.b_eff = ptr(m._eps_in), ptr(m._eps_out), ptr(m._w_eff), ptr(m._b_eff)
            self._noisy_desc_arr, self._noisy_desc_key = arr, key
        return self._noisy_desc_arr

    def _fuse_h_images(self):
        if not self._flat.is_cuda or PRECISION["fwd"] == "fp32" or PRECISION["bwd"] != "bf16":
            return False
        self._ensure_tc_buffers()
        return True

    def compose_weights(self):
        self._param_version += 1
        self._compose_weights()

    def _compose_weights(self):
        for _, module in self.noisy_layers():
            module._compose()
        self._refresh_tc_operands(force=True)
        self._composed_training = self.training

    def _live_weights_key(self):
        return (getattr(self, "_noise_version", 0), self._param_version, getattr(self, "_composed_training", None))

    def _ensure_tc_buffers(self):
        dev = self._flat.device
        if getattr(self, "_w_hi", None) is None or self._w_hi.device != dev:
            n = 2 * self.hidden
            mk = lambda *sh: torch.empty(*sh, dtype=torch.bfloat16, device=dev)
            self._w_hi, self._w_lo = mk(n, FEAT), mk(n, FEAT)
            self._w_hiT, self._w_loT = mk(FEAT, n), mk(FEAT, n)
            self._conv_ops = {}
            self._static_ops_dirty = True
            for name, conv in (("conv1", self.conv1), ("conv2", self.conv2), ("conv3", self.conv3)):
                co, k = conv.weight.shape[0], conv.weight[0].numel()
                self._conv_ops[name] = (mk(co, k), mk(co, k), mk(k, co))
            if self._embeds():
                self._iqn_ops = (mk(FEAT, self.quantile_embedding_dim), mk(FEAT, self.quantile_embedding_dim))

    def _refresh_tc_operands(self, force=False, h_done=False):
        if (PRECISION["fwd"] == "fp32" and PRECISION["bwd"] == "fp32") or not self._flat.is_cuda:
            return
        self._ensure_tc_buffers()
        dev = self._flat.device
        need_t = PRECISION["bwd"] != "bf16" or PRECISION["fwd"] == "fp32"
        if not h_done:
            f16 = PRECISION["fwd"] == "fp16"
            call("riqn_split_bf16", 2 * self.hidden, FEAT, ptr(self._w_eff_h), ptr(self._w_hi), ptr(self._w_lo),
                 ptr(self._w_hiT) if need_t else None, ptr(self._w_loT) if need_t else None, 1 if f16 else 0)
        if not (force or getattr(self, "_static_ops_dirty", True)):
            return
        self._static_ops_dirty = False
        if getattr(self, "_strip_ops", None) is None or self._strip_ops["conv1"][0].device != dev:
            self._strip_perm = {n: _strip_perm(cin, k, st, first).to(dev) for n, cin, k, st, first in
                                (("conv1", self.history, 8, 4, True), ("conv2", 32, 4, 2, False), ("conv3", 64, 3, 1, False))}
            self._strip_perm32 = {n: pm.to(torch.int32) for n, pm in self._strip_perm.items()}
            self._strip_ops = {n: (torch.empty(co, pm.numel(), dtype=torch.bfloat16, device=dev),
                                   torch.empty(co, pm.numel(), dtype=torch.bfloat16, device=dev))
                               for (n, pm), co in zip(self._strip_perm.items(), (32, 64, 64))}
            self._split_jobs = None
        convs = (("conv1", self.conv1), ("conv2", self.conv2), ("conv3", self.conv3))
        key = tuple(c.weight.data_ptr() for _, c in convs) + (self._strip_ops["conv1"][0].data_ptr(),)
        if getattr(self, "_split_jobs", None) is None or self._split_jobs[0] != key:
            specs = []
            for name, conv in convs:
                hi, lo, hiT = self._conv_ops[name]
                specs.append((conv.weight, None, 1.0, hi, lo, hiT))
                shi, slo = self._strip_ops[name]
                specs.append((conv.weight, self._strip_perm32[name], 255.0 if name == "conv1" else 1.0, shi, slo, None))
            if self._embeds():
                specs.append((self.iqn_fc.weight, None, 1.0, self._iqn_ops[0], self._iqn_ops[1], None))
            arr = (SplitJob * len(specs))()
            for j, (src, perm, div, hi, lo, hiT) in zip(arr, specs):
                j.src, j.perm = src.data_ptr(), perm.data_ptr() if perm is not None else None
                j.rows, j.cols, j.div = hi.shape[0], hi.shape[1], div
                j.hi, j.lo, j.hi_t = hi.data_ptr(), lo.data_ptr(), hiT.data_ptr() if hiT is not None else None
            self._split_jobs = (key, arr, len(specs))
        call("riqn_split_bf16_multi", self._split_jobs[2], self._split_jobs[1])

    def _support(self, dev):
        if getattr(self, "_support_t", None) is None or self._support_t.device != dev:
            self._support_t = torch.linspace(self._v_min, self._v_max, self.atoms).to(dev)
        return self._support_t

    def begin_step(self, dyn=None):
        self._dyn = dyn
        self._tau_in_step = self._shift_in_step = 0
        for _, m in self.noisy_layers():
            m._dyn = dyn
            m._calls_in_step = 0

    def draw_quantiles(self, n, risk=None):
        risk = check_risk(risk)
        tau = torch.empty(n, 1, device=self._flat.device)
        dyn = getattr(self, "_dyn", None)
        idx = self._tau_in_step if dyn is not None else self._tau_calls
        stream_id = self._tau_stream_offset + idx + (0 if dyn is not None else _EAGER_STREAMS)
        if risk is None:
            call("riqn_fill_uniform", n, self._rng_seed ^ 0x7A75, stream_id, ptr(tau), dyn.ptr() if dyn else None)
        else:
            call("riqn_fill_tau_distorted", n, self._rng_seed ^ 0x7A75, stream_id, RISK_MEASURES[risk[0]], risk[1], ptr(tau),
                 dyn.ptr() if dyn else None)
        self._tau_calls += 1
        self._tau_in_step += 1
        return tau

    def trunk(self, x, keep=None, col_cache=None):
        _lib.require_device()
        B = x.shape[0]
        if x.dtype not in (torch.uint8, torch.float32):
            x = x.float()
        if x.stride()[1:] != (84 * 84, 84, 1):
            x = x.contiguous()
        is_u8 = 1 if x.dtype == torch.uint8 else 0
        dev = x.device
        geoms, convs = self._trunk_geoms(B, x.stride(0)), (self.conv1, self.conv2, self.conv3)
        outs = (torch.empty(B, 32, 20, 20, device=dev), torch.empty(B, 64, 9, 9, device=dev),
                torch.empty(B, 64, 7, 7, device=dev))
        ins = (x, outs[0], outs[1])
        fwd = PRECISION["fwd"]
        bwd_tc = keep is not None and PRECISION["bwd"] == "bf16" and fwd != "fp32" and all((g.B * g.OH * g.OW) % 8 == 0 for g in geoms)
        cols, colTs = [None] * 3, [None] * 3
        strip_bwd = None
        if self._strip_ok(x):
            _, blocks = self._strip_trunk(x, outs if keep is not None else (None, None, outs[2]), col_cache=col_cache)
            if bwd_tc:
                strip_bwd = blocks
        elif fwd == "fp32":
            for i, (g, conv, inp, out) in enumerate(zip(geoms, convs, ins, outs)):
                cols[i] = torch.empty(g.B * g.OH * g.OW, g.Cin * g.KH * g.KW, device=dev)
                call("riqn_conv_fwd", g, ptr(inp), is_u8 if i == 0 else 0, ptr(conv.weight), ptr(conv.bias), ptr(cols[i]),
                     ptr(out))
        else:
            x3 = _small_x3()
            for i, (g, conv, inp, out) in enumerate(zip(geoms, convs, ins, outs)):
                M, K = g.B * g.OH * g.OW, g.Cin * g.KH * g.KW
                w_hi, w_lo, _ = self._conv_ops["conv%d" % (i + 1)]
                col_hi = torch.empty(M, K, dtype=torch.bfloat16, device=dev)
                col_lo = torch.empty(M, K, dtype=torch.bfloat16, device=dev) if x3 else None
                if bwd_tc:
                    colTs[i] = torch.empty(K, M, dtype=torch.bfloat16, device=dev)
                call("riqn_conv_fwd_tc", g, ptr(inp), is_u8 if i == 0 else 0, ptr(w_hi), ptr(w_lo), ptr(conv.bias),
                     ptr(col_hi), ptr(col_lo), ptr(colTs[i]), ptr(out))
        if keep is not None:
            if not bwd_tc and fwd != "fp32":
                for i, (g, inp) in enumerate(zip(geoms, ins)):
                    cols[i] = torch.empty(g.B * g.OH * g.OW, g.Cin * g.KH * g.KW, device=dev)
                    call("riqn_im2col_f32", g, ptr(inp), is_u8 if i == 0 else 0, ptr(cols[i]))
            keep.update(x=x, g=geoms, col=tuple(cols), colT=tuple(colTs), out=outs, bwd_tc=bwd_tc, strip_bwd=strip_bwd)
        return outs[2].view(B, FEAT)

    def _trunk_geoms(self, B, in_bstride=None):
        return (_geom(B, self.history, 84, 32, 8, 4, 1, in_bstride), _geom(B, 32, 20, 64, 4, 2, 0),
                _geom(B, 64, 9, 64, 3, 1, 0))

    def _strip_ok(self, x):
        return (PRECISION["fwd"] != "fp32" and x.dtype == torch.uint8 and x.stride()[1:] == (84 * 84, 84, 1)
                and x.stride(0) % 16 == 0 and x.data_ptr() % 16 == 0 and self.history == 4)

    def _strip_trunk(self, x, outs=None, other=None, col_cache=None):
        B, dev, x3 = x.shape[0], x.device, _small_x3()
        bf = lambda rows, cols: torch.empty(rows, cols, dtype=torch.bfloat16, device=dev)
        key = (x.data_ptr(), tuple(x.shape), tuple(x.stride()))
        a1 = col_cache.get(key) if col_cache is not None else None
        if a1 is None:
            g1 = self._trunk_geoms(B, x.stride(0))[0]
            G, width = _strip_block(g1)
            a1 = bf(B * G * G, width)
            call("riqn_s2d_u8", g1, ptr(x), ptr(a1))
            if col_cache is not None:
                col_cache[key] = a1

        def weights(net, name):
            hi, lo = net._strip_ops[name]
            return ptr(hi), ptr(lo) if x3 else None, ptr(getattr(net, name).bias)

        geoms = self._trunk_geoms(B if other is None else 2 * B)
        blocks, layouts = [(a1, None)], []
        for g in geoms[1:]:
            G, width = _strip_block(g)
            blocks.append((bf(g.B * G * G, width), bf(g.B * G * G, width) if x3 else None))
            layouts.append((g.stride, G))
        blocks.append((None, None))
        layouts.append((0, 0))
        if outs is None:
            outs = (None, None, torch.empty(geoms[2].B, FEAT, device=dev))
        for i, (name, g, out) in enumerate(zip(("conv1", "conv2", "conv3"), geoms, outs)):
            w2 = weights(other, name) if other is not None else (None, None, None)
            call("riqn_conv_fwd_strip", g, ptr(blocks[i][0]), ptr(blocks[i][1]), *weights(self, name), ptr(out),
                 ptr(blocks[i + 1][0]), ptr(blocks[i + 1][1]), *layouts[i], *w2, 1 if other is not None and i == 0 else 0)
        return outs[2].view(-1, FEAT), tuple(hi for hi, _ in blocks[:3])

    def trunk_pair(self, other, x):
        B = x.shape[0]
        if B % 128 or not (self._strip_ok(x) and other._strip_ok(x)):
            return None
        for net in (self, other):
            if getattr(net, "_strip_ops", None) is None or getattr(net, "_static_ops_dirty", True):
                net._refresh_tc_operands(h_done=True)
        feat, _ = self._strip_trunk(x, other=other)
        return feat[:B], feat[B:]

    def iqn_head(self, feat, num_quantiles, tau, keep=None):
        B = feat.shape[0]
        R = B * num_quantiles
        dev = feat.device
        E, hid, A = self.quantile_embedding_dim, self.hidden, self.action_space
        fwd, bwd = PRECISION["fwd"], PRECISION["bwd"]
        bf = lambda *sh: torch.empty(*sh, dtype=torch.bfloat16, device=dev)
        h = torch.empty(R, 2 * hid, device=dev)
        bwd_tc = keep is not None and bwd != "fp32" and R % 8 == 0
        emb_tc = keep is not None and bwd == "bf16" and fwd != "fp32" and R % 8 == 0
        cosv = xt = tc = None
        if fwd == "fp32":
            cosv = torch.empty(R, E, device=dev)
            xt = torch.empty(R, FEAT, device=dev)
            call("riqn_quantile_embed_fwd", B, num_quantiles, E, FEAT, ptr(tau), ptr(feat), ptr(self.iqn_fc.weight),
                 ptr(self.iqn_fc.bias), ptr(cosv), ptr(xt))
            if bwd_tc:
                tc = dict(x_hi=None, x_lo=None, x_hiT=bf(FEAT, R), x_loT=bf(FEAT, R) if bwd == "bf16x3" else None)
                call("riqn_split_bf16", R, FEAT, ptr(xt), None, None, ptr(tc["x_hiT"]), ptr(tc["x_loT"]), 0)
            call("riqn_noisy_linear_fwd", R, FEAT, 2 * hid, ptr(xt), ptr(self._w_eff_h), ptr(self._b_eff_h), ptr(h))
        else:
            x3 = _small_x3()
            f16 = fwd == "fp16"
            head_x3 = fwd == "bf16x3"
            need_x32 = keep is not None and not emb_tc
            mn = bwd_tc and bwd == "bf16"
            tc = dict(x_hi=torch.empty(R, FEAT, dtype=torch.float16 if f16 else torch.bfloat16, device=dev),
                      x_lo=bf(R, FEAT) if (head_x3 or (f16 and keep is not None)) else None, f16=f16,
                      x_hiT=bf(FEAT, R) if (bwd_tc and not mn) else None,
                      x_loT=bf(FEAT, R) if (bwd_tc and bwd == "bf16x3") else None,
                      cos_hi=bf(R, E), cos_lo=bf(R, E) if x3 else None, cosT_hi=None, mn=mn)
            if need_x32:
                xt = torch.empty(R, FEAT, device=dev)
                cosv = torch.empty(R, E, device=dev)
            elif tc["x_hiT"] is not None:
                xt = torch.empty(R, FEAT, device=dev)
            call("riqn_quantile_embed_fwd_tc", B, num_quantiles, E, FEAT, ptr(tau), ptr(feat), ptr(self._iqn_ops[0]),
                 ptr(self._iqn_ops[1]), ptr(self.iqn_fc.bias), ptr(tc["cos_hi"]), ptr(tc["cos_lo"]), ptr(tc["cosT_hi"]),
                 ptr(xt), ptr(tc["x_hi"]), ptr(tc["x_lo"]), ptr(tc["x_hiT"]), ptr(tc["x_loT"]), 1 if f16 else 0)
            if need_x32:
                call("riqn_quantile_embed_fwd", B, num_quantiles, E, FEAT, ptr(tau), ptr(feat), ptr(self.iqn_fc.weight),
                     ptr(self.iqn_fc.bias), ptr(cosv), ptr(xt))
            tc["h_hi"] = bf(R, 2 * hid) if (bwd_tc and R % 2 == 0) else None
            call("riqn_gemm_bf16_tc", R, 2 * hid, FEAT, ptr(tc["x_hi"]), ptr(tc["x_lo"]) if head_x3 else None, ptr(self._w_hi),
                 ptr(self._w_lo) if head_x3 else None, ptr(h), 2 * hid, 1, ptr(self._b_eff_h), None, None, 1, None, ptr(tc["h_hi"]),
                 3 if f16 else 0)
        q = torch.empty(R, A, device=dev)
        call("riqn_dueling_fwd", R, B, hid, A, ptr(h), ptr(self._w_eff_z), ptr(self._b_eff_z), ptr(q))
        if keep is not None:
            keep.update(feat=feat, cos=cosv, xt=xt, h=h, q=q, tau=tau, num_quantiles=num_quantiles, tc=tc,
                        noise_version=getattr(self, "_noise_version", 0),
                        head_bwd_tc=bwd_tc, emb_bwd_tc=emb_tc)
        return q

    def __call__(self, x, num_quantiles=None, log=False, tau=None, risk=None, **internal):
        if not internal and torch.is_grad_enabled() and any(p.requires_grad for p in self.parameters()):
            for name, t in (("x", x), ("tau", tau)):
                if torch.is_tensor(t) and t.requires_grad:
                    raise RuntimeError(f"DQN.forward computes gradients for the network's parameters only, not for its "
                                       f"inputs: {name} requires grad (pass {name}.detach())")
            params = [p for p in self.parameters() if p.requires_grad]
            return _DQNForward.apply(self, x, num_quantiles, log, tau, risk, *params)
        if risk is not None:
            internal["risk"] = risk
        return super().__call__(x, num_quantiles, log, tau, **internal)

    def forward(self, x, num_quantiles=None, log=False, tau=None, keep=None, fresh_weights=False, col_cache=None, feat=None,
                risk=None):
        if self.qr_dqn:
            bad = [f"{k}={v!r}" for k, v, ok in (("tau", tau, tau is None), ("risk", risk, risk is None),
                                                 ("log", log, not log),
                                                 ("num_quantiles", num_quantiles, num_quantiles in (None, self.num_quantiles)))
                   if not ok]
            if bad:
                raise ValueError(f"the QR-DQN network has N = {self.num_quantiles} fixed quantile fractions and no "
                                 f"log output: {', '.join(bad)} is not taken")
            from . import qr
            if keep is not None and feat is not None and not _trunk_kept(keep, feat):
                feat = None
            q = qr.forward(self, x, keep=keep, fresh_weights=fresh_weights, col_cache=col_cache, feat=feat)
            return q, qr.fractions(self, q.shape[0] // self.num_quantiles).clone()
        risk = check_risk(risk)
        if self.rainbow_only:
            if risk is not None:
                raise ValueError("risk measures distort the IQN quantile fractions; the C51 network acts risk-neutrally")
            from . import c51
            return c51.forward(self, x, log=log, keep=keep, fresh_weights=fresh_weights)
        if not fresh_weights:
            self._compose_weights()
        if feat is None or (keep is not None and not _trunk_kept(keep, feat)):
            feat = self.trunk(x, keep, col_cache)
        if tau is None:
            tau = self.draw_quantiles(num_quantiles * x.shape[0], risk)
        else:
            tau = tau.to(feat.device, torch.float32).reshape(-1, 1).contiguous()
        q = self.iqn_head(feat, num_quantiles, tau, keep)
        return q, tau

    def backward_iqn(self, keep, dtheta, gscale, actions, gscale_mul=1.0):
        if keep.get("noise_version", None) != getattr(self, "_noise_version", 0):
            raise RuntimeError("the network's noise was resampled between this forward pass and its backward: the composed "
                               "weights / epsilons of the gradient pass are gone (call backward before the next reset_noise)")
        R, B, hid, A = keep["feat"].shape[0] * keep["num_quantiles"], keep["feat"].shape[0], self.hidden, self.action_space

        def one_hot(fused_dh, dh, dh_hi, dbs, dz, dzT):
            if fused_dh:
                call("riqn_dueling_bwd_bf16", R, B, hid, A, ptr(keep["h"]), ptr(keep["tc"].get("h_hi")), ptr(self._w_eff_z),
                     ptr(dtheta), ptr(gscale), float(gscale_mul), ptr(actions), ptr(dh_hi), None, ptr(dbs), ptr(dz), ptr(dzT))
            else:
                call("riqn_dueling_bwd", R, B, hid, A, ptr(keep["h"]), ptr(self._w_eff_z), ptr(dtheta), ptr(gscale),
                     float(gscale_mul), ptr(actions), ptr(dh), ptr(dz), ptr(dzT))
        self._backward_head(keep, one_hot, self.grad_view)

    def backward_iqn_dense(self, keep, grad_q, gv=None):
        R, B, hid, A = keep["feat"].shape[0] * keep["num_quantiles"], keep["feat"].shape[0], self.hidden, self.action_space

        def dense(fused_dh, dh, dh_hi, dbs, dz, dzT):
            if fused_dh:
                call("riqn_dueling_bwd_dense_bf16", R, B, hid, A, ptr(keep["h"]), ptr(keep["tc"].get("h_hi")),
                     ptr(self._w_eff_z), ptr(grad_q), ptr(dh_hi), None, ptr(dbs), ptr(dz), ptr(dzT))
            else:
                call("riqn_dueling_bwd_dense", R, B, hid, A, ptr(keep["h"]), ptr(self._w_eff_z), ptr(grad_q), ptr(dh),
                     ptr(dz), ptr(dzT))
        self._backward_head(keep, dense, gv or self.grad_view)

    def _backward_head(self, keep, dueling_bwd, gv):
        B = keep["feat"].shape[0]
        Nq = keep["num_quantiles"]
        R = B * Nq
        dev = keep["feat"].device
        hid, A, E = self.hidden, self.action_space, self.quantile_embedding_dim
        hv, ha, zv, za = self.fcnoisy_h_v, self.fcnoisy_h_a, self.fcnoisy_z_v, self.fcnoisy_z_a
        dz = torch.empty(R, 32, device=dev)
        tc = keep.get("tc")
        f16 = bool(tc and tc.get("f16"))
        x_bf = tc["x_lo"] if f16 else (tc["x_hi"] if tc else None)
        w_bf = self._w_lo if f16 else getattr(self, "_w_hi", None)
        z_tc = bool(keep["head_bwd_tc"]) and tc is not None and tc.get("h_hi") is not None
        dzT = torch.empty(R, 32, dtype=torch.bfloat16, device=dev) if z_tc else None
        dbs = torch.empty(2 * hid, device=dev)
        fused_dh = bool(keep["head_bwd_tc"]) and PRECISION["bwd"] == "bf16" and R % 8 == 0 and bool(tc and tc.get("mn"))
        if fused_dh:
            dh = None
            dh_hi = torch.empty(R, 2 * hid, dtype=torch.bfloat16, device=dev)
            dh_hiT = None
        else:
            dh, dh_hi = torch.empty(R, 2 * hid, device=dev), None
        dueling_bwd(fused_dh, dh, dh_hi, dbs, dz, dzT)
        dwz = torch.empty(32, 2 * hid, device=dev)
        dbz = torch.empty(32, device=dev)
        zargs = (ptr(dwz), ptr(dbz), ptr(zv.weight_epsilon), ptr(zv.bias_epsilon), ptr(za.weight_epsilon),
                 ptr(za.bias_epsilon), ptr(gv(zv.weight_mu)), ptr(gv(zv.weight_sigma)), ptr(gv(zv.bias_mu)),
                 ptr(gv(zv.bias_sigma)), ptr(gv(za.weight_mu)), ptr(gv(za.weight_sigma)), ptr(gv(za.bias_mu)),
                 ptr(gv(za.bias_sigma)))
        if z_tc:
            call("riqn_z_wgrad_tc", R, hid, A, ptr(dzT), ptr(tc["h_hi"]), ptr(dz), *zargs)
        else:
            call("riqn_z_wgrad", R, hid, A, ptr(dz), ptr(keep["h"]), *zargs)
        bwd = PRECISION["bwd"]
        dx_bf16 = fused_dh and bool(keep["emb_bwd_tc"])
        dx = torch.empty(R, FEAT, dtype=torch.bfloat16 if dx_bf16 else torch.float32, device=dev)
        if not keep["head_bwd_tc"]:
            call("riqn_noisy_linear_wgrad", R, FEAT, 2 * hid, ptr(dh), ptr(keep["xt"]), ptr(hv.weight_epsilon),
                 ptr(hv.bias_epsilon), ptr(dbs), ptr(gv(hv.weight_mu)), ptr(gv(hv.weight_sigma)), ptr(gv(hv.bias_mu)),
                 ptr(gv(hv.bias_sigma)))
            call("riqn_noisy_linear_dgrad", R, FEAT, 2 * hid, ptr(dh), ptr(self._w_eff_h), ptr(dx))
        else:
            bf = lambda *sh: torch.empty(*sh, dtype=torch.bfloat16, device=dev)
            b3 = bwd == "bf16x3"
            dh_lo, dh_loT = (bf(R, 2 * hid), bf(2 * hid, R)) if b3 else (None, None)
            if not fused_dh:
                dh_hi, dh_hiT = bf(R, 2 * hid), bf(2 * hid, R)
                call("riqn_split_bf16", R, 2 * hid, ptr(dh), ptr(dh_hi), ptr(dh_lo), ptr(dh_hiT), ptr(dh_loT), 0)
            if fused_dh:
                call("riqn_gemm_bf16_tc_mn", 2 * hid, FEAT, R, ptr(dh_hi), ptr(x_bf), 1, ptr(gv(hv.weight_mu)), FEAT, 3,
                     ptr(gv(hv.weight_sigma)), ptr(hv.weight_epsilon), 1.0, WGRAD_SPLIT_K, None, 0)
            else:
                call("riqn_gemm_bf16_tc", 2 * hid, FEAT, R, ptr(dh_hiT), ptr(dh_loT), ptr(tc["x_hiT"]),
                     ptr(tc["x_loT"]) if b3 else None, ptr(gv(hv.weight_mu)), FEAT, 3, None, ptr(gv(hv.weight_sigma)),
                     ptr(hv.weight_epsilon), WGRAD_SPLIT_K, None, None, 0)
            call("riqn_noisy_bias_grad", R, 2 * hid, ptr(dh) if dh is not None else None, ptr(hv.bias_epsilon), ptr(dbs),
                 ptr(gv(hv.bias_mu)), ptr(gv(hv.bias_sigma)))
            hook = getattr(self, "_grads_ready_hook", None)
            if hook is not None:
                hook(self._offsets[id(hv.weight_mu)])
            if fused_dh:
                call("riqn_gemm_bf16_tc_mn", R, FEAT, 2 * hid, ptr(dh_hi), ptr(w_bf), 0, None if dx_bf16 else ptr(dx), FEAT,
                     0, None, None, 1.0, 1, ptr(dx) if dx_bf16 else None, 0)
            else:
                call("riqn_gemm_bf16_tc", R, FEAT, 2 * hid, ptr(dh_hi), ptr(dh_lo), ptr(self._w_hiT),
                     ptr(self._w_loT) if b3 else None, ptr(dx), FEAT, 0, None, None, None, 1, None, None, 0)
        dfeat = torch.empty(B, FEAT, device=dev)
        if keep["emb_bwd_tc"]:
            dpre = torch.empty(R, FEAT, dtype=torch.bfloat16, device=dev)
            call("riqn_quantile_embed_bwd_tc", B, Nq, E, FEAT, ptr(x_bf), None if (dx_bf16 or f16) else ptr(tc["x_lo"]),
                 ptr(keep["feat"]), ptr(tc["cos_hi"]), ptr(dx), 1 if dx_bf16 else 0, ptr(dpre), ptr(dfeat),
                 ptr(gv(self.iqn_fc.weight)), ptr(gv(self.iqn_fc.bias)))
        else:
            call("riqn_quantile_embed_bwd", B, Nq, E, FEAT, ptr(keep["xt"]), ptr(keep["feat"]), ptr(keep["cos"]), ptr(dx),
                 ptr(dfeat), ptr(gv(self.iqn_fc.weight)), ptr(gv(self.iqn_fc.bias)))
        self.backward_trunk(keep, dfeat)

    def backward_trunk(self, keep, dfeat):
        (g1, g2, g3), (out1, out2, out3) = keep["g"], keep["out"]
        dev = dfeat.device
        gv = self.grad_view
        convs = (self.conv1, self.conv2, self.conv3)
        douts = [None, None, dfeat]
        for i in (2, 1, 0):
            g, conv, out = keep["g"][i], convs[i], keep["out"][i]
            M, K = g.B * g.OH * g.OW, g.Cin * g.KH * g.KW
            din = torch.empty_like(keep["out"][i - 1]) if i > 0 else None
            if keep["bwd_tc"] and keep.get("strip_bwd") is not None:
                name = "conv%d" % (i + 1)
                w_hi = self._conv_ops[name][0]
                G, _ = _strip_block(g)
                dYg = torch.empty(g.B * G * G, g.Cout, dtype=torch.bfloat16, device=dev)
                dwp = torch.empty(g.Cout, K, device=dev)
                call("riqn_conv_bwd_strip", g, ptr(douts[i]), ptr(out), ptr(keep["strip_bwd"][i]), ptr(w_hi),
                     ptr(self._strip_perm32[name]), ptr(dYg), ptr(dwp), ptr(gv(conv.weight)), ptr(gv(conv.bias)), ptr(din),
                     1.0 / 255.0 if i == 0 else 1.0)
            elif keep["bwd_tc"]:
                _, _, wT_hi = self._conv_ops["conv%d" % (i + 1)]
                dY = torch.empty(M, g.Cout, dtype=torch.bfloat16, device=dev) if i > 0 else None
                dYT = torch.empty(g.Cout, M, dtype=torch.bfloat16, device=dev)
                dcol = torch.empty(M, K, device=dev) if i > 0 else None
                call("riqn_conv_bwd_tc", g, ptr(douts[i]), ptr(out), ptr(keep["colT"][i]), ptr(wT_hi), ptr(dY), ptr(dYT),
                     ptr(dcol), ptr(gv(conv.weight)), ptr(gv(conv.bias)), ptr(din), 1.0)
            else:
                dY = torch.empty(M, g.Cout, device=dev)
                dcol = torch.empty(M, K, device=dev) if i > 0 else None
                call("riqn_conv_bwd", g, ptr(douts[i]), ptr(out), ptr(keep["col"][i]), ptr(conv.weight), ptr(dY), ptr(dcol),
                     ptr(gv(conv.weight)), ptr(gv(conv.bias)), ptr(din))
            if i > 0:
                douts[i - 1] = din


def _trunk_kept(keep, feat):
    out = keep.get("out")
    return out is not None and out[2].data_ptr() == feat.data_ptr() and out[2].numel() == feat.numel()


def _grad_views(net, training):
    if training:
        return net.grad_view
    scratch = torch.empty_like(net._flat_grad)
    sigmas = {id(p) for _, m in net.noisy_layers() for p in (m.weight_sigma, m.bias_sigma)}

    def gv(p):
        off = net._offsets[id(p)]
        return (scratch if id(p) in sigmas else net._flat_grad)[off:off + p.numel()].view(p.shape)
    return gv


class _DQNForward(torch.autograd.Function):

    @staticmethod
    def forward(ctx, net, x, num_quantiles, log, tau, risk, *params):
        keep = {}
        out = net.forward(x, num_quantiles, log, tau, keep, risk=risk)
        ctx.net, ctx.keep, ctx.log, ctx.n_params = net, keep, log, len(params)
        ctx.live = net._live_weights_key()
        if net.rainbow_only:
            ctx.save_for_backward(out)
            return out
        if net.qr_dqn:
            q, tau = out
            ctx.mark_non_differentiable(tau)
            return q, tau
        keep.pop("q")
        keep.pop("tau")
        q, tau = out
        ctx.mark_non_differentiable(tau)
        return q, tau

    @staticmethod
    @torch.autograd.function.once_differentiable
    def backward(ctx, grad_out, *_):
        net, keep = ctx.net, ctx.keep
        if keep is None:
            raise RuntimeError("backward through this DQN forward already ran: its saved state is released after the first "
                               "backward (run the forward again for a second backward)")
        if net._live_weights_key() != ctx.live:
            raise RuntimeError("the network's weights changed between this forward and its backward (reset_noise(), an "
                               "optimiser step, load_state_dict(), compose_weights() or a train/eval switch with a new "
                               "forward): the backward reads the live weights, so call it before such a change")
        ctx.keep = None
        gv = _grad_views(net, ctx.live[2])
        g = grad_out.contiguous().float()
        if net.rainbow_only:
            from . import c51
            out, = ctx.saved_tensors
            c51.backward_dense(net, keep, out, g, ctx.log, gv)
        elif net.qr_dqn:
            from . import qr
            qr.backward_dense(net, keep, g, gv)
        else:
            net.backward_iqn_dense(keep, g, gv)
        return (None,) * (6 + ctx.n_params)


class _NoisyLinearFn(torch.autograd.Function):

    @staticmethod
    def forward(ctx, layer, input, weight_mu, weight_sigma, bias_mu, bias_sigma):
        x = input.contiguous().float()
        out = layer._forward(x)
        ctx.save_for_backward(x, layer._w_eff.clone(), layer.weight_epsilon.clone(), layer.bias_epsilon.clone())
        ctx.training, ctx.in_dtype = layer.training, input.dtype
        return out

    @staticmethod
    @torch.autograd.function.once_differentiable
    def backward(ctx, grad_out):
        x, w_eff, eps_w, eps_b = ctx.saved_tensors
        dy = grad_out.contiguous().float()
        rows, n_in, n_out = x.shape[0], w_eff.shape[1], w_eff.shape[0]
        dx = None
        if ctx.needs_input_grad[1]:
            dx = torch.empty_like(x)
            call("riqn_noisy_linear_dgrad", rows, n_in, n_out, ptr(dy), ptr(w_eff), ptr(dx))
            dx = dx.to(ctx.in_dtype)
        g_wmu, g_wsig = torch.zeros_like(w_eff), torch.zeros_like(w_eff)
        g_bmu, g_bsig = torch.zeros(n_out, device=x.device), torch.zeros(n_out, device=x.device)
        db = torch.empty(n_out, device=x.device)
        call("riqn_noisy_linear_wgrad", rows, n_in, n_out, ptr(dy), ptr(x), ptr(eps_w), ptr(eps_b), ptr(db), ptr(g_wmu),
             ptr(g_wsig), ptr(g_bmu), ptr(g_bsig))
        if not ctx.training:
            g_wsig = g_bsig = None
        return None, dx, g_wmu, g_wsig, g_bmu, g_bsig
```

### rainbow_iqn_apex_b200/qr.py

```python
import numbers

import torch

from . import c51
from ._lib import call, ptr
from .compute_loss_iqn import _as_device_inputs, _quantile_loss, greedy_actions

MAX_QUANTILES = 256
MAX_ACTIONS = 32


def check_qr(qr_dqn, num_tau_samples=None, action_space=None, rainbow_only=False, munchausen=None, fqf=None, risk=None):
    if isinstance(qr_dqn, bool) or (isinstance(qr_dqn, numbers.Integral) and qr_dqn in (0, 1)):
        if not qr_dqn:
            return None
    else:
        raise ValueError(f"qr_dqn must be 0 or 1, got {qr_dqn!r}")
    if (isinstance(num_tau_samples, bool) or not isinstance(num_tau_samples, numbers.Integral)
            or not 2 <= num_tau_samples <= MAX_QUANTILES):
        raise ValueError(f"QR-DQN needs num_tau_samples (its N) in 2..{MAX_QUANTILES}, got {num_tau_samples!r}")
    if action_space is not None and not 1 <= action_space <= MAX_ACTIONS:
        raise ValueError(f"QR-DQN supports 1..{MAX_ACTIONS} actions, got {action_space!r}")
    if rainbow_only:
        raise ValueError("qr_dqn and rainbow_only are two different heads on the same network: set one of them")
    if munchausen is not None:
        raise ValueError("QR-DQN and Munchausen targets do not combine: set munchausen = 0 or qr_dqn = 0")
    if fqf is not None:
        raise ValueError("QR-DQN has fixed fractions and FQF learned ones: set fqf = 0 or qr_dqn = 0")
    if risk is not None:
        raise ValueError("QR-DQN has fixed quantile fractions: a risk measure has nothing to distort; use the neutral "
                         "measure")
    return int(num_tau_samples)


def fractions(net, batch):
    N, dev = net.num_quantiles, net._flat.device
    cache = net.__dict__.setdefault("_qr_tau", {})
    t = cache.get(batch)
    if t is None or t.device != dev:
        i = torch.arange(N, dtype=torch.float32)
        tau = (2.0 * i + 1.0) / float(2 * N)
        t = tau.repeat_interleave(batch).reshape(N * batch, 1).to(dev)
        cache[batch] = t
    return t


def forward(net, x, keep=None, fresh_weights=False, col_cache=None, feat=None):
    if not fresh_weights:
        net._compose_weights()
    zv, za = c51.hidden_z(net, x, keep=keep, col_cache=col_cache, feat=feat)
    B, A, N = zv.shape[0], net.action_space, net.num_quantiles
    q = torch.empty(N * B, A, device=zv.device)
    call("riqn_qr_head_fwd", B, A, N, ptr(zv), ptr(za), ptr(q))
    return q


def backward_dense(on, keep, grad_q, gv):
    B, N = keep["B"], on.num_quantiles
    dzv = torch.empty(B, N, device=grad_q.device)
    dza = torch.empty(B, on.action_space * N, device=grad_q.device)
    call("riqn_qr_head_bwd_dense", B, on.action_space, N, ptr(grad_q), ptr(dzv), ptr(dza))
    c51._backward_below_head(on, keep, dzv, dza, gv)


def loss_core(agent, states, actions, returns, next_states, nonterminals, debug=None):
    states, actions, returns, next_states, nonterminals = _as_device_inputs(
        agent, states, actions, returns, next_states, nonterminals)
    on, tg = agent.online_net, agent.target_net
    B, A, N = states.shape[0], agent.action_space, agent.num_tau_samples
    dev = states.device
    inj = getattr(agent, "_inject", None)
    if isinstance(inj, list):
        inj = inj.pop(0) if inj else None
    noises = inj.get("noises", (None, None, None)) if inj else (None, None, None)
    on.reset_noise(noises[0])
    cache = {}
    pair = on.trunk_pair(tg, next_states)
    f_on, f_tg = pair if pair is not None else (None, None)
    q_sel = forward(on, next_states, fresh_weights=True, col_cache=cache, feat=f_on)
    a_star = greedy_actions(agent, B, N, q_sel)
    tg.reset_noise(noises[1])
    q_tgt = forward(tg, next_states, fresh_weights=True, col_cache=cache, feat=f_tg)
    on.reset_noise(noises[2])
    keep = {}
    q_on = forward(on, states, keep=keep, fresh_weights=True)
    tau_hat = fractions(on, B)
    loss = torch.empty(B, device=dev)
    dtheta = torch.empty(N * B, device=dev)
    theta_out = target_out = None
    if debug is not None:
        theta_out = torch.empty(B, N, device=dev)
        target_out = torch.empty(B, N, device=dev)
    _quantile_loss(agent, B, N, N, q_on, q_tgt, tau_hat, actions, a_star, returns, nonterminals, loss, dtheta, theta_out,
                   target_out)
    if debug is not None:
        debug.update(a_star=a_star, theta=theta_out, target=target_out, q_sel=q_sel, q_tgt=q_tgt, q_on=q_on,
                     tau=tau_hat, keep=keep)
    version = getattr(on, "_noise_version", 0)

    def backward(gscale, gscale_mul=1.0):
        if getattr(on, "_noise_version", 0) != version:
            raise RuntimeError("the online network's noise was resampled between the QR-DQN loss and its backward")
        gscale = gscale.contiguous().float()
        dzv = torch.empty(B, N, device=dev)
        dza = torch.empty(B, A * N, device=dev)
        call("riqn_qr_head_bwd", B, A, N, ptr(dtheta), ptr(gscale), float(gscale_mul), ptr(actions), ptr(dzv), ptr(dza))
        c51._backward_below_head(on, keep, dzv, dza, on.grad_view)

    return loss, backward


def compute_loss_qr(agent, states, actions, returns, next_states, nonterminals, debug=None):
    if torch.is_grad_enabled():
        params = [p for p in agent.online_net.parameters() if p.requires_grad]
        return c51._HeadLoss.apply(loss_core, agent, states, actions, returns, next_states, nonterminals, debug, *params)
    loss, _ = loss_core(agent, states, actions, returns, next_states, nonterminals, debug=debug)
    return loss
```

Before: 275.0.

## Fuse the three-layer conv trunk forward into one persistent wgmma kernel

Replaces the per-layer strip conv launches and the separate space-to-depth pass with a single persistent kernel. Each block loads raw uint8 frames into shared memory, builds the conv1 operands in registers, and runs conv1, conv2 and conv3 with wgmma. Weight slabs stream through a cp.async ring buffer, and both nets of the online/target pair can be processed in one launch. This removes the global-memory round trips of intermediate activations and several kernel launches, and drops the col_cache reuse path. In exchange the kernel is hard-wired to 84x84x4 Atari geometry, uses large shared memory with one block per SM, and only writes the layer activations needed for backward when gradients are required.

```diff
diff --git a/include/riqn_b200.h b/include/riqn_b200.h
--- a/include/riqn_b200.h
+++ b/include/riqn_b200.h
@@ -43,6 +43,13 @@
 int riqn_conv_fwd_strip(const riqn_conv_geom* g, const void* a_hi, const void* a_lo, const void* w_hi, const void* w_lo,
                         const float* bias, float* out, void* next_hi, void* next_lo, int next_stride, int next_grid,
                         const void* w2_hi, const void* w2_lo, const float* bias2, int share_a, void* stream);
+typedef struct riqn_trunk_weights {
+  const void* hi[3];
+  const void* lo[3];
+  const float* bias[3];
+} riqn_trunk_weights;
+int riqn_trunk_fwd_fused(const riqn_conv_geom* g, const unsigned char* frames, const riqn_trunk_weights* w, int n_sets,
+                         float* feat, void* a1, void* a2_hi, void* a3_hi, float* out1, float* out2, void* stream);
 int riqn_conv_bwd_strip(const riqn_conv_geom* g, const float* dout, const float* out, const void* a_hi, const void* w_hi,
                         const int* perm, void* dYg, float* dwp_scratch, float* dw, float* dbias, float* din,
                         float wgrad_scale, void* stream);
diff --git a/rainbow_iqn_apex_b200/_lib.py b/rainbow_iqn_apex_b200/_lib.py
--- a/rainbow_iqn_apex_b200/_lib.py
+++ b/rainbow_iqn_apex_b200/_lib.py
@@ -28,6 +28,10 @@
                 ("lo", _P), ("hi_t", _P)]
 
 
+class TrunkWeights(C.Structure):
+    _fields_ = [("hi", _P * 3), ("lo", _P * 3), ("bias", _P * 3)]
+
+
 SIGNATURES = {
     "riqn_version": [],
     "riqn_device_ok": [],
@@ -40,6 +44,7 @@
     "riqn_s2d_u8": [C.POINTER(ConvGeom), _P, _P, _P],
     "riqn_conv_fwd_strip": [C.POINTER(ConvGeom), _P, _P, _P, _P, _P, _P, _P, _P, C.c_int, C.c_int, _P, _P, _P, C.c_int, _P],
     "riqn_conv_bwd_strip": [C.POINTER(ConvGeom), _P, _P, _P, _P, _P, _P, _P, _P, _P, _P, C.c_float, _P],
+    "riqn_trunk_fwd_fused": [C.POINTER(ConvGeom), _P, C.POINTER(TrunkWeights), C.c_int, _P, _P, _P, _P, _P, _P, _P],
     "riqn_split_bf16_scaled": [C.c_long, C.c_int, _P, C.c_float, _P, _P, _P],
     "riqn_fill_uniform": [C.c_long, C.c_ulonglong, C.c_ulonglong, _P, _P, _P],
     "riqn_fill_tau_distorted": [C.c_long, C.c_ulonglong, C.c_ulonglong, C.c_int, C.c_float, _P, _P, _P],
diff --git a/rainbow_iqn_apex_b200/c51.py b/rainbow_iqn_apex_b200/c51.py
--- a/rainbow_iqn_apex_b200/c51.py
+++ b/rainbow_iqn_apex_b200/c51.py
@@ -22,10 +22,10 @@
     return out
 
 
-def hidden_z(net, x, keep=None, col_cache=None, feat=None):
+def hidden_z(net, x, keep=None, feat=None):
     from .model import PRECISION
     if feat is None:
-        feat = net.trunk(x, keep, col_cache)
+        feat = net.trunk(x, keep)
     B = feat.shape[0]
     dev = feat.device
     hid = net.hidden
diff --git a/rainbow_iqn_apex_b200/compute_loss_iqn.py b/rainbow_iqn_apex_b200/compute_loss_iqn.py
--- a/rainbow_iqn_apex_b200/compute_loss_iqn.py
+++ b/rainbow_iqn_apex_b200/compute_loss_iqn.py
@@ -105,14 +105,13 @@
         return _fqf_core(agent, states, actions, returns, next_states, nonterminals, noises, keep_graph, debug)
 
     on.reset_noise(noises[0])
-    cache = {}
     pair = on.trunk_pair(tg, next_states) if not on.rainbow_only else None
     f_on, f_tg = pair if pair is not None else (None, None)
-    q_sel, tau_sel = on.forward(next_states, K, tau=taus[0], fresh_weights=True, col_cache=cache, feat=f_on,
+    q_sel, tau_sel = on.forward(next_states, K, tau=taus[0], fresh_weights=True, feat=f_on,
                                 risk=getattr(agent, "risk", None))
     a_star = greedy_actions(agent, B, K, q_sel)
     tg.reset_noise(noises[1])
-    q_tgt, _ = tg.forward(next_states, Np, tau=taus[1], fresh_weights=True, col_cache=cache, feat=f_tg)
+    q_tgt, _ = tg.forward(next_states, Np, tau=taus[1], fresh_weights=True, feat=f_tg)
     on.reset_noise(noises[2])
     keep = {} if keep_graph else None
     q_on, tau = on.forward(states, N, tau=taus[2], keep=keep, fresh_weights=True)
@@ -163,17 +162,16 @@
     B, N = states.shape[0], agent.num_tau_samples
     dev = states.device
     on.reset_noise(noises[0])
-    cache = {}
     pair = on.trunk_pair(tg, next_states)
-    f_on, f_tg = pair if pair is not None else (on.trunk(next_states, col_cache=cache), None)
+    f_on, f_tg = pair if pair is not None else (on.trunk(next_states), None)
     fr_n = fnet.propose(f_on)
-    q_sel, _ = on.forward(next_states, N, tau=fr_n["tau_hat"], fresh_weights=True, col_cache=cache, feat=f_on)
+    q_sel, _ = on.forward(next_states, N, tau=fr_n["tau_hat"], fresh_weights=True, feat=f_on)
     a_star = greedy_actions(agent, B, N, q_sel, fr_n["dtau"])
     keep = {} if keep_graph else None
     feat = on.trunk(states, keep)
     fr = fnet.propose(feat)
     tg.reset_noise(noises[1])
-    q_tgt, _ = tg.forward(next_states, N, tau=fr["tau_hat"], fresh_weights=True, col_cache=cache, feat=f_tg)
+    q_tgt, _ = tg.forward(next_states, N, tau=fr["tau_hat"], fresh_weights=True, feat=f_tg)
     on.reset_noise(noises[2])
     q_on, tau_hat = on.forward(states, N, tau=fr["tau_hat"], keep=keep, fresh_weights=True, feat=feat)
     nb = N - 1 if (N - 1) * B % 2 == 0 else N
diff --git a/rainbow_iqn_apex_b200/csrc/conv.cu b/rainbow_iqn_apex_b200/csrc/conv.cu
--- a/rainbow_iqn_apex_b200/csrc/conv.cu
+++ b/rainbow_iqn_apex_b200/csrc/conv.cu
@@ -415,6 +415,328 @@
 static inline int grid_for(long total) {
   long b = (total + 255) / 256;
   return (int)(b > 32L * riqn_sms() ? 32L * riqn_sms() : (b < 1 ? 1 : b));
+}
+
+constexpr int kFzThreads = 512;
+constexpr int kFzFrame = 4 * 84 * 84;
+constexpr int kFzSlots = 4, kFzSlabs = 19;
+constexpr uint32_t kFzSlot = 16384;
+constexpr uint32_t kFzX = 28672, kFzSample = kFzX + 2 * 100 * 256;
+constexpr uint32_t kFzSmem = kFzSlots * kFzSlot + 2 * kFzSample + 1024;
+constexpr int kFzG1 = 21, kFzG2 = 10, kFzG3 = 9;
+
+__device__ __forceinline__ uint64_t fz_desc_k128(uint32_t saddr) {
+  return (uint64_t)((saddr & 0x3FFFF) >> 4) | ((uint64_t)1 << 16) | ((uint64_t)(1024 >> 4) << 32) | ((uint64_t)1 << 62);
+}
+__device__ __forceinline__ void fz_wgmma_fence() { asm volatile("wgmma.fence.sync.aligned;" ::: "memory"); }
+__device__ __forceinline__ void fz_wgmma_commit_wait() {
+  asm volatile("wgmma.commit_group.sync.aligned;" ::: "memory");
+  asm volatile("wgmma.wait_group.sync.aligned 0;" ::: "memory");
+}
+
+template <int N>
+__device__ __forceinline__ void fz_wgmma(float (&d)[N / 2], const uint32_t (&a)[4], uint64_t db, uint32_t acc);
+template <>
+__device__ __forceinline__ void fz_wgmma<32>(float (&d)[16], const uint32_t (&a)[4], uint64_t db, uint32_t acc) {
+  asm volatile(
+      "{\n.reg .pred p;\nsetp.ne.b32 p, %21, 0;\n"
+      "wgmma.mma_async.sync.aligned.m64n32k16.f32.bf16.bf16 "
+      "{%0, %1, %2, %3, %4, %5, %6, %7, %8, %9, %10, %11, %12, %13, %14, %15}, {%16, %17, %18, %19}, %20, p, 1, 1, 0;\n}\n"
+      : "+f"(d[0]), "+f"(d[1]), "+f"(d[2]), "+f"(d[3]), "+f"(d[4]), "+f"(d[5]), "+f"(d[6]), "+f"(d[7]),
+        "+f"(d[8]), "+f"(d[9]), "+f"(d[10]), "+f"(d[11]), "+f"(d[12]), "+f"(d[13]), "+f"(d[14]), "+f"(d[15])
+      : "r"(a[0]), "r"(a[1]), "r"(a[2]), "r"(a[3]), "l"(db), "r"(acc));
+}
+template <>
+__device__ __forceinline__ void fz_wgmma<64>(float (&d)[32], const uint32_t (&a)[4], uint64_t db, uint32_t acc) {
+  asm volatile(
+      "{\n.reg .pred p;\nsetp.ne.b32 p, %37, 0;\n"
+      "wgmma.mma_async.sync.aligned.m64n64k16.f32.bf16.bf16 "
+      "{%0, %1, %2, %3, %4, %5, %6, %7, %8, %9, %10, %11, %12, %13, %14, %15, %16, %17, %18, %19, %20, %21, %22, %23, "
+      "%24, %25, %26, %27, %28, %29, %30, %31}, {%32, %33, %34, %35}, %36, p, 1, 1, 0;\n}\n"
+      : "+f"(d[0]), "+f"(d[1]), "+f"(d[2]), "+f"(d[3]), "+f"(d[4]), "+f"(d[5]), "+f"(d[6]), "+f"(d[7]),
+        "+f"(d[8]), "+f"(d[9]), "+f"(d[10]), "+f"(d[11]), "+f"(d[12]), "+f"(d[13]), "+f"(d[14]), "+f"(d[15]),
+        "+f"(d[16]), "+f"(d[17]), "+f"(d[18]), "+f"(d[19]), "+f"(d[20]), "+f"(d[21]), "+f"(d[22]), "+f"(d[23]),
+        "+f"(d[24]), "+f"(d[25]), "+f"(d[26]), "+f"(d[27]), "+f"(d[28]), "+f"(d[29]), "+f"(d[30]), "+f"(d[31])
+      : "r"(a[0]), "r"(a[1]), "r"(a[2]), "r"(a[3]), "l"(db), "r"(acc));
+}
+
+__device__ __forceinline__ void fz_ldmatrix_x4(uint32_t (&a)[4], uint32_t addr) {
+  asm volatile("ldmatrix.sync.aligned.m8n8.x4.shared.b16 {%0, %1, %2, %3}, [%4];"
+               : "=r"(a[0]), "=r"(a[1]), "=r"(a[2]), "=r"(a[3]) : "r"(addr) : "memory");
+}
+__device__ __forceinline__ void fz_cp16(uint32_t dst, const void* src) {
+  asm volatile("cp.async.cg.shared.global [%0], [%1], 16;" ::"r"(dst), "l"(src) : "memory");
+}
+__device__ __forceinline__ void fz_cp_commit() { asm volatile("cp.async.commit_group;" ::: "memory"); }
+template <int N>
+__device__ __forceinline__ void fz_cp_wait() { asm volatile("cp.async.wait_group %0;" ::"n"(N) : "memory"); }
+
+__device__ __forceinline__ void fz_split(float x0, float x1, uint32_t& hi, uint32_t& lo) {
+  const __nv_bfloat162 h = __floats2bfloat162_rn(x0, x1);
+  hi = *reinterpret_cast<const uint32_t*>(&h);
+  const __nv_bfloat162 l = __floats2bfloat162_rn(x0 - __uint_as_float(hi << 16), x1 - __uint_as_float(hi & 0xffff0000u));
+  lo = *reinterpret_cast<const uint32_t*>(&l);
+}
+
+struct FzArgs {
+  const uint8_t* frames;
+  long bstride;
+  int B;
+  int units_per_set, units;
+  riqn_trunk_weights w[2];
+  float* feat;
+  bf16 *a1, *a2, *a3;
+  float *out1, *out2;
+};
+
+template <bool X3>
+__device__ __forceinline__ void fz_issue(const FzArgs& p, uint32_t wbuf, long q) {
+  const long it = q / kFzSlabs;
+  const int pos = (int)(q - it * kFzSlabs);
+  const long unit = blockIdx.x + it * gridDim.x;
+  if (unit < p.units) {
+    const bool s1 = unit >= p.units_per_set;
+    const uint32_t dst = wbuf + (uint32_t)(q % kFzSlots) * kFzSlot;
+    const int i = threadIdx.x, n = (i >> 3) & 63, j = i & 7;
+    if (pos < 2) {
+      const int kk = i >> 8, nn = n & 31, kb = 2 * pos + kk;
+      const uint32_t d = dst + kk * 8192 + nn * 128 + ((j ^ (nn & 7)) << 4);
+      const long src = (long)nn * 256 + kb * 64 + j * 8;
+      fz_cp16(d, (const bf16*)(s1 ? p.w[1].hi[0] : p.w[0].hi[0]) + src);
+      if (X3) fz_cp16(d + 4096, (const bf16*)(s1 ? p.w[1].lo[0] : p.w[0].lo[0]) + src);
+    } else {
+      const int l = pos < 10 ? 1 : 2, kb = pos - (pos < 10 ? 2 : 10), K = l == 1 ? 512 : 576;
+      const uint32_t d = dst + n * 128 + ((j ^ (n & 7)) << 4);
+      const long src = (long)n * K + kb * 64 + j * 8;
+      const void* hi = l == 1 ? (s1 ? p.w[1].hi[1] : p.w[0].hi[1]) : (s1 ? p.w[1].hi[2] : p.w[0].hi[2]);
+      fz_cp16(d, (const bf16*)hi + src);
+      if (X3) {
+        const void* lo = l == 1 ? (s1 ? p.w[1].lo[1] : p.w[0].lo[1]) : (s1 ? p.w[1].lo[2] : p.w[0].lo[2]);
+        fz_cp16(d + 8192, (const bf16*)lo + src);
+      }
+    }
+  }
+  fz_cp_commit();
+}
+
+template <bool X3, int T, int KC, int G, int P>
+__device__ __forceinline__ void fz_layer64(const FzArgs& p, float (&acc)[32], uint32_t a_hi, uint32_t lo_off,
+                                           uint32_t wbuf, long& q, int tile, int warp_in_wg, int lane) {
+  constexpr int KB = T * T * KC, ROWS = G * G;
+  const int r_lane = tile * 64 + 16 * warp_in_wg + (lane & 15);
+  for (int kb = 0; kb < KB; ++kb, ++q) {
+    fz_cp_wait<kFzSlots - 2>();
+    __syncthreads();
+    fz_issue<X3>(p, wbuf, q + kFzSlots - 1);
+    const uint32_t slot = wbuf + (uint32_t)(q % kFzSlots) * kFzSlot;
+    const int s = kb / KC, dy = s / T, dx = s - dy * T;
+    int r = r_lane + dy * G + dx;
+    r = r < ROWS ? r : ROWS - 1;
+    const uint32_t rbase = a_hi + r * P;
+    uint32_t fh[4][4], fl[4][4];
+#pragma unroll
+    for (int k = 0; k < 4; ++k) {
+      const int piece = (kb - s * KC) * 8 + 2 * k + (lane >> 4);
+      const uint32_t addr = rbase + ((piece ^ (r & 7)) << 4);
+      fz_ldmatrix_x4(fh[k], addr);
+      if (X3) fz_ldmatrix_x4(fl[k], addr + lo_off);
+    }
+    fz_wgmma_fence();
+#pragma unroll
+    for (int k = 0; k < 4; ++k) {
+      const uint64_t bh = fz_desc_k128(slot + k * 32);
+      fz_wgmma<64>(acc, fh[k], bh, (kb > 0 || k > 0) ? 1u : 0u);
+      if (X3) {
+        fz_wgmma<64>(acc, fh[k], fz_desc_k128(slot + 8192 + k * 32), 1u);
+        fz_wgmma<64>(acc, fl[k], bh, 1u);
+      }
+    }
+    fz_wgmma_commit_wait();
+  }
+}
+
+template <bool X3, bool GRAD>
+__global__ void __launch_bounds__(kFzThreads, 1) trunk_fwd_fused_kernel(const __grid_constant__ FzArgs p) {
+  extern __shared__ uint8_t fz_raw[];
+  uint8_t* sm = reinterpret_cast<uint8_t*>((reinterpret_cast<uintptr_t>(fz_raw) + 1023) & ~uintptr_t(1023));
+  const uint32_t sbase = (uint32_t)__cvta_generic_to_shared(sm);
+  const uint32_t wbuf = sbase;
+  constexpr uint32_t kLo2 = 100 * 256, kLo3 = 81 * 128;
+  const int tid = threadIdx.x, lane = tid & 31, wg = tid >> 7, wq = (tid >> 5) & 3;
+  const int sub = wg >> 1, wg2 = wg & 1, lt = tid & 255;
+  const int fr = 16 * wq + (lane >> 2), fc = 2 * (lane & 3);
+  const uint32_t x_off = kFzSlots * kFzSlot + sub * kFzSample;
+  const uint8_t* img = sm + x_off;
+  const uint32_t x_s = sbase + x_off, y_s = x_s + kFzX;
+  long q = 0;
+  for (int i = 0; i < kFzSlots - 1; ++i) fz_issue<X3>(p, wbuf, i);
+  for (long unit = blockIdx.x; unit < p.units; unit += gridDim.x) {
+    const int set = unit >= p.units_per_set ? 1 : 0;
+    const int first = (int)(unit - set * p.units_per_set) * 2, fb = first + sub;
+    const bool live = fb < p.B;
+    const long smp = (long)set * p.B + fb;
+    const float* bias1 = set ? p.w[1].bias[0] : p.w[0].bias[0];
+    const float* bias2 = set ? p.w[1].bias[1] : p.w[0].bias[1];
+    const float* bias3 = set ? p.w[1].bias[2] : p.w[0].bias[2];
+    for (int s = 0; s < 2; ++s) {
+      if (first + s >= p.B) break;
+      const uint4* src = reinterpret_cast<const uint4*>(p.frames + (long)(first + s) * p.bstride);
+      uint4* dst = reinterpret_cast<uint4*>(sm + kFzSlots * kFzSlot + s * kFzSample);
+      for (int i = tid; i < kFzFrame / 16; i += kFzThreads) dst[i] = src[i];
+    }
+    fz_cp_wait<kFzSlots - 3>();
+    __syncthreads();
+    fz_issue<X3>(p, wbuf, q + kFzSlots - 1);
+    const uint32_t c1[2] = {wbuf + (uint32_t)(q % kFzSlots) * kFzSlot, wbuf + (uint32_t)((q + 1) % kFzSlots) * kFzSlot};
+    if (GRAD && live) {
+      bf16* dst = p.a1 + (long)fb * kFzG1 * kFzG1 * 64;
+      for (int it = lt; it < kFzG1 * kFzG1 * 8; it += 256) {
+        const int r = it >> 3, j8 = it & 7, gy = r / kFzG1, gx = r - gy * kFzG1;
+        uint32_t e[8];
+#pragma unroll
+        for (int t = 0; t < 8; ++t) {
+          const int k = j8 * 8 + t, c = k >> 4, iy = (k >> 2) & 3, ix = k & 3;
+          const int y = gy * 4 + iy - 1, x = gx * 4 + ix - 1;
+          e[t] = ((unsigned)y < 84u && (unsigned)x < 84u) ? __float_as_uint((float)img[(c * 84 + y) * 84 + x]) >> 16 : 0u;
+        }
+        *reinterpret_cast<uint4*>(dst + r * 64 + j8 * 8) =
+            make_uint4(e[0] | (e[1] << 16), e[2] | (e[3] << 16), e[4] | (e[5] << 16), e[6] | (e[7] << 16));
+      }
+    }
+    {
+      float b1[8];
+#pragma unroll
+      for (int j = 0; j < 4; ++j) { b1[2 * j] = __ldg(bias1 + 8 * j + fc); b1[2 * j + 1] = __ldg(bias1 + 8 * j + fc + 1); }
+      for (int tile = wg2; tile < 7; tile += 2) {
+        float acc[16];
+        int gy2[2], gx2[2];
+#pragma unroll
+        for (int h = 0; h < 2; ++h) {
+          const int m = tile * 64 + fr + 8 * h;
+          gy2[h] = m / kFzG1;
+          gx2[h] = m - gy2[h] * kFzG1;
+        }
+#pragma unroll
+        for (int kb = 0; kb < 4; ++kb) {
+          const int dy = kb >> 1, dx = kb & 1;
+          uint32_t fa[4][4];
+#pragma unroll
+          for (int h = 0; h < 2; ++h) {
+            const int x0 = 4 * (gx2[h] + dx) - 1 + 2 * (lane & 1);
+#pragma unroll
+            for (int hy = 0; hy < 2; ++hy) {
+              const int y = 4 * (gy2[h] + dy) - 1 + ((lane & 3) >> 1) + 2 * hy;
+              const bool ok0 = (unsigned)y < 84u && (unsigned)x0 < 84u, ok1 = (unsigned)y < 84u && (unsigned)(x0 + 1) < 84u;
+#pragma unroll
+              for (int c = 0; c < 4; ++c) {
+                const uint8_t* row = img + (c * 84 + y) * 84;
+                const uint32_t v0 = ok0 ? __float_as_uint((float)row[x0]) >> 16 : 0u;
+                const uint32_t v1 = ok1 ? __float_as_uint((float)row[x0 + 1]) >> 16 : 0u;
+                fa[c][2 * hy + h] = v0 | (v1 << 16);
+              }
+            }
+          }
+          fz_wgmma_fence();
+          const uint32_t slot = c1[kb >> 1] + (kb & 1) * 8192;
+#pragma unroll
+          for (int k = 0; k < 4; ++k) {
+            fz_wgmma<32>(acc, fa[k], fz_desc_k128(slot + k * 32), (kb > 0 || k > 0) ? 1u : 0u);
+            if (X3) fz_wgmma<32>(acc, fa[k], fz_desc_k128(slot + 4096 + k * 32), 1u);
+          }
+          fz_wgmma_commit_wait();
+        }
+#pragma unroll
+        for (int h = 0; h < 2; ++h) {
+          const int m = tile * 64 + fr + 8 * h, gy = gy2[h], gx = gx2[h];
+          if (m >= kFzG1 * kFzG1 || gy >= 20 || gx >= 20) continue;
+          const int r2 = (gy >> 1) * kFzG2 + (gx >> 1), cb = ((gy & 1) * 2 + (gx & 1)) * 32;
+#pragma unroll
+          for (int j = 0; j < 4; ++j) {
+            const int n = 8 * j + fc;
+            const float x0 = fmaxf(acc[4 * j + 2 * h] + b1[2 * j], 0.f), x1 = fmaxf(acc[4 * j + 2 * h + 1] + b1[2 * j + 1], 0.f);
+            uint32_t hi, lo;
+            fz_split(x0, x1, hi, lo);
+            const int col = cb + n;
+            const uint32_t off = r2 * 256 + ((((col >> 3) ^ (r2 & 7))) << 4) + (col & 7) * 2;
+            asm volatile("st.shared.b32 [%0], %1;" ::"r"(y_s + off), "r"(hi) : "memory");
+            asm volatile("st.shared.b32 [%0], %1;" ::"r"(y_s + kLo2 + off), "r"(lo) : "memory");
+            if (GRAD && live) {
+              float* o = p.out1 + (((long)fb * 32 + n) * 20 + gy) * 20 + gx;
+              o[0] = x0;
+              o[400] = x1;
+            }
+          }
+        }
+      }
+    }
+    __syncthreads();
+    fz_issue<X3>(p, wbuf, q + kFzSlots);
+    q += 2;
+    if (GRAD && live) {
+      bf16* dst = p.a2 + (long)fb * 100 * 128;
+      for (int it = lt; it < 100 * 16; it += 256) {
+        const int r = it >> 4, j = it & 15;
+        const uint4 v = *reinterpret_cast<const uint4*>(sm + x_off + kFzX + r * 256 + ((j ^ (r & 7)) << 4));
+        *reinterpret_cast<uint4*>(dst + r * 128 + j * 8) = v;
+      }
+    }
+    {
+      float acc[32];
+      fz_layer64<X3, 2, 2, kFzG2, 256>(p, acc, y_s, kLo2, wbuf, q, wg2, wq, lane);
+      float b2[16];
+#pragma unroll
+      for (int j = 0; j < 8; ++j) { b2[2 * j] = __ldg(bias2 + 8 * j + fc); b2[2 * j + 1] = __ldg(bias2 + 8 * j + fc + 1); }
+#pragma unroll
+      for (int h = 0; h < 2; ++h) {
+        const int m = wg2 * 64 + fr + 8 * h, gy = m / kFzG2, gx = m - gy * kFzG2;
+        if (m >= 100 || gy >= 9 || gx >= 9) continue;
+        const int r3 = gy * kFzG3 + gx;
+#pragma unroll
+        for (int j = 0; j < 8; ++j) {
+          const int n = 8 * j + fc;
+          const float x0 = fmaxf(acc[4 * j + 2 * h] + b2[2 * j], 0.f), x1 = fmaxf(acc[4 * j + 2 * h + 1] + b2[2 * j + 1], 0.f);
+          uint32_t hi, lo;
+          fz_split(x0, x1, hi, lo);
+          const uint32_t off = r3 * 128 + (((n >> 3) ^ (r3 & 7)) << 4) + (n & 7) * 2;
+          asm volatile("st.shared.b32 [%0], %1;" ::"r"(x_s + off), "r"(hi) : "memory");
+          asm volatile("st.shared.b32 [%0], %1;" ::"r"(x_s + kLo3 + off), "r"(lo) : "memory");
+          if (GRAD && live) {
+            float* o = p.out2 + (((long)fb * 64 + n) * 9 + gy) * 9 + gx;
+            o[0] = x0;
+            o[81] = x1;
+          }
+        }
+      }
+    }
+    {
+      float acc[32];
+      fz_layer64<X3, 3, 1, kFzG3, 128>(p, acc, x_s, kLo3, wbuf, q, wg2, wq, lane);
+      if (GRAD && live) {
+        bf16* dst = p.a3 + (long)fb * 81 * 64;
+        for (int it = lt; it < 81 * 8; it += 256) {
+          const int r = it >> 3, j = it & 7;
+          const uint4 v = *reinterpret_cast<const uint4*>(sm + x_off + r * 128 + ((j ^ (r & 7)) << 4));
+          *reinterpret_cast<uint4*>(dst + r * 64 + j * 8) = v;
+        }
+      }
+      if (live) {
+        float* f = p.feat + smp * 3136;
+#pragma unroll
+        for (int h = 0; h < 2; ++h) {
+          const int m = wg2 * 64 + fr + 8 * h, gy = m / kFzG3, gx = m - gy * kFzG3;
+          if (m >= 81 || gy >= 7 || gx >= 7) continue;
+#pragma unroll
+          for (int j = 0; j < 8; ++j) {
+            const int n = 8 * j + fc;
+            f[n * 49 + gy * 7 + gx] = fmaxf(acc[4 * j + 2 * h] + __ldg(bias3 + n), 0.f);
+            f[(n + 1) * 49 + gy * 7 + gx] = fmaxf(acc[4 * j + 2 * h + 1] + __ldg(bias3 + n + 1), 0.f);
+          }
+        }
+      }
+    }
+    __syncthreads();
+  }
+  fz_cp_wait<0>();
 }
 
 }
@@ -629,6 +951,44 @@
   ex.nx_hi = (bf16*)next_hi; ex.nx_lo = (bf16*)next_lo; ex.nx_s = next_stride; ex.nx_G = next_grid;
   return gemm_bf16_tc(g->B * G * G, g->Cout, g->Cin * g->KH * g->KW, (const bf16*)a_hi, (const bf16*)a_lo, (const bf16*)w_hi,
                       (const bf16*)w_lo, out, g->Cout, TC_CONV, bias, nullptr, nullptr, 1, (cudaStream_t)stream, &ex);
+}
+
+RIQN_API int riqn_trunk_fwd_fused(const riqn_conv_geom* g, const unsigned char* frames, const riqn_trunk_weights* w,
+                                  int n_sets, float* feat, void* a1, void* a2_hi, void* a3_hi, float* out1, float* out2,
+                                  void* stream) {
+  riqn::note_launches(1);
+  const bool grad = a1 != nullptr;
+  if (g == nullptr || w == nullptr || feat == nullptr || g->B < 1 || g->Cin != 4 || g->H != 84 || g->W != 84 ||
+      g->Cout != 32 || g->KH != 8 || g->KW != 8 || g->stride != 4 || g->pad != 1 || g->OH != 20 || g->OW != 20 ||
+      g->in_bstride % 16 || g->in_bstride < kFzFrame || (reinterpret_cast<uintptr_t>(frames) & 15) ||
+      (n_sets != 1 && n_sets != 2) || (grad && (n_sets != 1 || !a2_hi || !a3_hi || !out1 || !out2)) ||
+      (!grad && (a2_hi || a3_hi || out1 || out2)))
+    return (int)cudaErrorInvalidValue;
+  const bool x3 = w[0].lo[0] != nullptr;
+  for (int s = 0; s < n_sets; ++s)
+    for (int l = 0; l < 3; ++l)
+      if (!w[s].hi[l] || !w[s].bias[l] || (w[s].lo[l] != nullptr) != x3) return (int)cudaErrorInvalidValue;
+  FzArgs p;
+  p.frames = frames; p.bstride = g->in_bstride; p.B = g->B;
+  p.units_per_set = (g->B + 1) / 2; p.units = p.units_per_set * n_sets;
+  p.w[0] = w[0]; p.w[1] = w[n_sets - 1];
+  p.feat = feat;
+  p.a1 = (bf16*)a1; p.a2 = (bf16*)a2_hi; p.a3 = (bf16*)a3_hi; p.out1 = out1; p.out2 = out2;
+  static PerDeviceOnce attr_once;
+  const int dev = PerDeviceOnce::device();
+  if (!attr_once.done[dev]) {
+    for (auto kernel : {trunk_fwd_fused_kernel<true, true>, trunk_fwd_fused_kernel<true, false>,
+                        trunk_fwd_fused_kernel<false, true>, trunk_fwd_fused_kernel<false, false>})
+      RIQN_CUDA(cudaFuncSetAttribute(kernel, cudaFuncAttributeMaxDynamicSharedMemorySize, (int)kFzSmem));
+    attr_once.done[dev] = true;
+  }
+  const auto go = [&](void (*kernel)(FzArgs)) -> int {
+    const long grid = std::min<long>(p.units, riqn_sms());
+    kernel<<<(int)grid, kFzThreads, kFzSmem, (cudaStream_t)stream>>>(p);
+    return (int)cudaGetLastError();
+  };
+  if (x3) return grad ? go(trunk_fwd_fused_kernel<true, true>) : go(trunk_fwd_fused_kernel<true, false>);
+  return grad ? go(trunk_fwd_fused_kernel<false, true>) : go(trunk_fwd_fused_kernel<false, false>);
 }
 
 RIQN_API int riqn_conv_bwd_strip(const riqn_conv_geom* g, const float* dout, const float* out, const void* a_hi,
diff --git a/rainbow_iqn_apex_b200/model.py b/rainbow_iqn_apex_b200/model.py
--- a/rainbow_iqn_apex_b200/model.py
+++ b/rainbow_iqn_apex_b200/model.py
@@ -468,7 +468,7 @@
         self._tau_in_step += 1
         return tau
 
-    def trunk(self, x, keep=None, col_cache=None):
+    def trunk(self, x, keep=None):
         _lib.require_device()
         B = x.shape[0]
         if x.dtype not in (torch.uint8, torch.float32):
@@ -486,7 +486,7 @@
         cols, colTs = [None] * 3, [None] * 3
         strip_bwd = None
         if self._strip_ok(x):
-            _, blocks = self._strip_trunk(x, outs if keep is not None else (None, None, outs[2]), col_cache=col_cache)
+            _, blocks = self._strip_trunk(x, outs if keep is not None else (None, None, outs[2]))
             if bwd_tc:
                 strip_bwd = blocks
         elif fwd == "fp32":
@@ -521,38 +521,23 @@
         return (PRECISION["fwd"] != "fp32" and x.dtype == torch.uint8 and x.stride()[1:] == (84 * 84, 84, 1)
                 and x.stride(0) % 16 == 0 and x.data_ptr() % 16 == 0 and self.history == 4)
 
-    def _strip_trunk(self, x, outs=None, other=None, col_cache=None):
+    def _strip_trunk(self, x, outs=None, other=None):
         B, dev, x3 = x.shape[0], x.device, _small_x3()
         bf = lambda rows, cols: torch.empty(rows, cols, dtype=torch.bfloat16, device=dev)
-        key = (x.data_ptr(), tuple(x.shape), tuple(x.stride()))
-        a1 = col_cache.get(key) if col_cache is not None else None
-        if a1 is None:
-            g1 = self._trunk_geoms(B, x.stride(0))[0]
-            G, width = _strip_block(g1)
-            a1 = bf(B * G * G, width)
-            call("riqn_s2d_u8", g1, ptr(x), ptr(a1))
-            if col_cache is not None:
-                col_cache[key] = a1
-
-        def weights(net, name):
-            hi, lo = net._strip_ops[name]
-            return ptr(hi), ptr(lo) if x3 else None, ptr(getattr(net, name).bias)
-
-        geoms = self._trunk_geoms(B if other is None else 2 * B)
-        blocks, layouts = [(a1, None)], []
-        for g in geoms[1:]:
-            G, width = _strip_block(g)
-            blocks.append((bf(g.B * G * G, width), bf(g.B * G * G, width) if x3 else None))
-            layouts.append((g.stride, G))
-        blocks.append((None, None))
-        layouts.append((0, 0))
+        nets = (self,) if other is None else (self, other)
+        sets = (_lib.TrunkWeights * len(nets))()
+        for s, net in zip(sets, nets):
+            for i, name in enumerate(("conv1", "conv2", "conv3")):
+                hi, lo = net._strip_ops[name]
+                s.hi[i], s.lo[i], s.bias[i] = hi.data_ptr(), lo.data_ptr() if x3 else None, getattr(net, name).bias.data_ptr()
+        geoms = self._trunk_geoms(B, x.stride(0))
+        grad = outs is not None and outs[0] is not None
+        blocks = tuple(bf(B * G * G, width) for G, width in map(_strip_block, geoms)) if grad else None
         if outs is None:
-            outs = (None, None, torch.empty(geoms[2].B, FEAT, device=dev))
-        for i, (name, g, out) in enumerate(zip(("conv1", "conv2", "conv3"), geoms, outs)):
-            w2 = weights(other, name) if other is not None else (None, None, None)
-            call("riqn_conv_fwd_strip", g, ptr(blocks[i][0]), ptr(blocks[i][1]), *weights(self, name), ptr(out),
-                 ptr(blocks[i + 1][0]), ptr(blocks[i + 1][1]), *layouts[i], *w2, 1 if other is not None and i == 0 else 0)
-        return outs[2].view(-1, FEAT), tuple(hi for hi, _ in blocks[:3])
+            outs = (None, None, torch.empty(B * len(nets), FEAT, device=dev))
+        call("riqn_trunk_fwd_fused", geoms[0], ptr(x), sets, len(nets), ptr(outs[2]),
+             *((ptr(a) for a in blocks) if grad else (None,) * 3), ptr(outs[0]), ptr(outs[1]))
+        return outs[2].view(-1, FEAT), blocks
 
     def trunk_pair(self, other, x):
         B = x.shape[0]
@@ -630,7 +615,7 @@
             internal["risk"] = risk
         return super().__call__(x, num_quantiles, log, tau, **internal)
 
-    def forward(self, x, num_quantiles=None, log=False, tau=None, keep=None, fresh_weights=False, col_cache=None, feat=None,
+    def forward(self, x, num_quantiles=None, log=False, tau=None, keep=None, fresh_weights=False, feat=None,
                 risk=None):
         if self.qr_dqn:
             bad = [f"{k}={v!r}" for k, v, ok in (("tau", tau, tau is None), ("risk", risk, risk is None),
@@ -643,7 +628,7 @@
             from . import qr
             if keep is not None and feat is not None and not _trunk_kept(keep, feat):
                 feat = None
-            q = qr.forward(self, x, keep=keep, fresh_weights=fresh_weights, col_cache=col_cache, feat=feat)
+            q = qr.forward(self, x, keep=keep, fresh_weights=fresh_weights, feat=feat)
             return q, qr.fractions(self, q.shape[0] // self.num_quantiles).clone()
         risk = check_risk(risk)
         if self.rainbow_only:
@@ -654,7 +639,7 @@
         if not fresh_weights:
             self._compose_weights()
         if feat is None or (keep is not None and not _trunk_kept(keep, feat)):
-            feat = self.trunk(x, keep, col_cache)
+            feat = self.trunk(x, keep)
         if tau is None:
             tau = self.draw_quantiles(num_quantiles * x.shape[0], risk)
         else:
diff --git a/rainbow_iqn_apex_b200/qr.py b/rainbow_iqn_apex_b200/qr.py
--- a/rainbow_iqn_apex_b200/qr.py
+++ b/rainbow_iqn_apex_b200/qr.py
@@ -45,10 +45,10 @@
     return t
 
 
-def forward(net, x, keep=None, fresh_weights=False, col_cache=None, feat=None):
+def forward(net, x, keep=None, fresh_weights=False, feat=None):
     if not fresh_weights:
         net._compose_weights()
-    zv, za = c51.hidden_z(net, x, keep=keep, col_cache=col_cache, feat=feat)
+    zv, za = c51.hidden_z(net, x, keep=keep, feat=feat)
     B, A, N = zv.shape[0], net.action_space, net.num_quantiles
     q = torch.empty(N * B, A, device=zv.device)
     call("riqn_qr_head_fwd", B, A, N, ptr(zv), ptr(za), ptr(q))
@@ -74,13 +74,12 @@
         inj = inj.pop(0) if inj else None
     noises = inj.get("noises", (None, None, None)) if inj else (None, None, None)
     on.reset_noise(noises[0])
-    cache = {}
     pair = on.trunk_pair(tg, next_states)
     f_on, f_tg = pair if pair is not None else (None, None)
-    q_sel = forward(on, next_states, fresh_weights=True, col_cache=cache, feat=f_on)
+    q_sel = forward(on, next_states, fresh_weights=True, feat=f_on)
     a_star = greedy_actions(agent, B, N, q_sel)
     tg.reset_noise(noises[1])
-    q_tgt = forward(tg, next_states, fresh_weights=True, col_cache=cache, feat=f_tg)
+    q_tgt = forward(tg, next_states, fresh_weights=True, feat=f_tg)
     on.reset_noise(noises[2])
     keep = {}
     q_on = forward(on, states, keep=keep, fresh_weights=True)
```

Result: slower. 267.5 (median of 6 runs) (-2.7%).
